# leonsick/s2d

Measured on AMD Instinct MI355X. Metric: clip-frames/sec fwd+loss, R50 M2F-Video T=8 720p Q=100, higher is better.
Workload: dtype f32 (f16x3 MFMA for dense contractions); 1 GPU; KDVideoMaskFormer fwd+loss (student+teacher fwd, GT+KD VideoSetCriterion), c4: 2 clips/GPU x T=8 x 720x1280, Q=100, P=160000, N=10 sparse GT instances/clip, encoder dropout 0.3; clips_per_gpu=2, frames_per_clip=8, parallelism=dp1 (clips sharded, no collective), streams=2

## Files before the change

### s2d_amd/csrc/ffn.hip

```cpp
#include "common.h"
#include "dropout.h"
#include <stdlib.h>
#include <type_traits>

#ifndef S2D_FFN_DBG
#define S2D_FFN_DBG 0
#endif
#if !(S2D_FFN_DBG & 16)
#define FFN_STAMP(slot) do { } while (0)
#endif
#ifndef S2D_FFN_EPI
#define S2D_FFN_EPI 1
#endif
#ifndef S2D_FFN_POSTV
#define S2D_FFN_POSTV 0
#endif

#if S2D_FFN_DBG & 16
__device__ unsigned long long g_ffn_stamps[16 * 4096];
#define FFN_STAMP(slot) do { if (tid == 0 && blockIdx.x < 4096) g_ffn_stamps[16 * blockIdx.x + (slot)] = __builtin_amdgcn_s_memtime(); } while (0)
extern "C" int s2d_ffn_dbg_stamps(unsigned long long *host_out)
{
    return hipMemcpyFromSymbol(host_out, HIP_SYMBOL(g_ffn_stamps), sizeof(g_ffn_stamps)) == hipSuccess ? 0 : -1;
}
#endif

namespace {

typedef _Float16 f16x8 __attribute__((ext_vector_type(8)));
typedef __fp16 h16x2 __attribute__((ext_vector_type(2)));
typedef float f32x2 __attribute__((ext_vector_type(2)));
typedef unsigned int u32x4 __attribute__((ext_vector_type(4)));

constexpr int FC = 256;
constexpr int FRAG = 1024;
constexpr int PART = 32 * FRAG;
constexpr int CHUNKB = 2 * PART;
constexpr int LDS_B1 = 2 * CHUNKB;
constexpr int FMAX = 2048;
constexpr int LDS_PB = LDS_B1 + FMAX * 4;
constexpr int LDS_LN = LDS_PB + FC * 4;

__host__ __device__ __forceinline__ int perm_row(int rho) { return 16 * ((rho >> 2) & 1) + 4 * (rho >> 3) + (rho & 3); }

__device__ __forceinline__ unsigned int pk_hi(float a, float b) { return __builtin_bit_cast(unsigned int, __builtin_amdgcn_cvt_pkrtz(a, b)); }
__device__ __forceinline__ unsigned int pk_lo(float a, float b, unsigned int hi)
{
    const h16x2 h = __builtin_bit_cast(h16x2, hi);
    return __builtin_bit_cast(unsigned int, __builtin_amdgcn_cvt_pkrtz(__builtin_fmaf((float)h[0], -2048.f, a * 2048.f), __builtin_fmaf((float)h[1], -2048.f, b * 2048.f)));
}

__device__ __forceinline__ int lane16_asm()
{
    int v;
    asm volatile("v_mbcnt_lo_u32_b32 %0, -1, 0\n\tv_mbcnt_hi_u32_b32 %0, -1, %0\n\tv_lshlrev_b32 %0, 4, %0" : "=v"(v));
    return v;
}
struct MfmaPrev { f16x8 a, b; };
__device__ __forceinline__ void mfma_a(f32x16 &c, const f16x8 a, const f16x8 b) { c = __builtin_amdgcn_mfma_f32_32x32x16_f16(a, b, c, 0, 0, 0); }
__device__ __forceinline__ void mfma_v(f32x16 &c, const f16x8 a, const f16x8 b, MfmaPrev &pv)
{
    asm("v_mfma_f32_32x32x16_f16 %0, %1, %2, %0" : "+v"(c) : "v"(a), "v"(b), "v"(pv.a), "v"(pv.b));
    pv.a = a; pv.b = b;
}
__device__ __forceinline__ void mfma_v0(f32x16 &c, const f16x8 a, const f16x8 b, MfmaPrev &pv)
{
    asm("v_mfma_f32_32x32x16_f16 %0, %1, %2, 0" : "=&v"(c) : "v"(a), "v"(b), "v"(pv.a), "v"(pv.b));
    pv.a = a; pv.b = b;
}

__host__ __device__ __forceinline__ int kcol(int ks, int h) { return 32 * (ks >> 1) + 16 * h + 8 * (ks & 1); }

__global__ __launch_bounds__(256) void ffn_pack_kernel(const float *__restrict__ W1, const float *__restrict__ W2, int F,
                                                       const float *__restrict__ Wpost, int npost, const float *__restrict__ Wpre, int npre,
                                                       u32x4 *__restrict__ out)
{
    const long gid = (long)blockIdx.x * 256 + threadIdx.x;
    const long nfrag = (long)(F / 32) * 64 + (long)((npost + npre) / 32) * 32;
    if (gid >= nfrag * 64) return;
    const int lane = (int)(gid & 63);
    const long fidx = gid >> 6;
    const int r = lane & 31, h = lane >> 5;
    const float *src;
    int lo;
    if (fidx < (long)(F / 32) * 64) {
        const int frag = (int)(fidx & 63);
        const long c = fidx >> 6;
        lo = frag & 1;
        if (frag < 32) src = W1 + (32 * c + perm_row(r)) * FC + kcol(frag >> 1, h);
        else {
            const int f2 = frag - 32, s = f2 >> 4, t = (f2 >> 1) & 7;
            src = W2 + (long)(32 * t + perm_row(r)) * F + 32 * c + 16 * h + 8 * s;
        }
    } else {
        const long f2 = fidx - (long)(F / 32) * 64;
        const int frag = (int)(f2 & 31);
        lo = frag & 1;
        const long part = f2 >> 5;
        src = (part < npost / 32 ? Wpost + (32 * part + perm_row(r)) * FC : Wpre + (32 * (part - npost / 32) + perm_row(r)) * FC) + kcol(frag >> 1, h);
    }
    u32x4 w;
#pragma unroll
    for (int q = 0; q < 4; ++q) {
        const unsigned int hi = pk_hi(src[2 * q], src[2 * q + 1]);
        w[q] = lo ? pk_lo(src[2 * q], src[2 * q + 1], hi) : hi;
    }
    out[gid] = w;
}

struct FfnParams {
    const float *X;
    float *Y;
    float *Xn;
    int M, nchunks;
    const unsigned int *pack;
    const float *b1, *b2;
    const float *g1, *be1;
    const float *g2, *be2;
    float eps;
    unsigned int thresh;
    float dscale;
    unsigned int k0, k1, site_h, site_o, row0;
    const float *post_bias, *post_pos;
    const float *pre_bias, *pre_res;
    unsigned int site_pre;
    float *post_out;
    int post_parts, post_S, post_npos, post_ld, post_ldpos;
};

template <bool DROP, bool LN1, bool LN2, bool POST, bool PRE>
__global__ __launch_bounds__(256) __attribute__((amdgpu_waves_per_eu(1, 1))) void ffn_f16x3_kernel(FfnParams p)
{
    extern __shared__ __attribute__((aligned(16))) unsigned char lds[];
    const int tid = threadIdx.x, lane = tid & 63, wave = __builtin_amdgcn_readfirstlane(tid >> 6);
#if S2D_FFN_DBG & 16
    const unsigned long long st_te = __builtin_amdgcn_s_memtime();
#endif
    const int tok = lane & 31, h = lane >> 5;
    const long row = (long)blockIdx.x * 128 + wave * 32 + tok;
    const bool rowok = row < p.M;
    const long rowc = rowok ? row : p.M - 1;
    const unsigned int mrow = p.row0 + (unsigned int)rowc;

    const __amdgpu_buffer_rsrc_t rsW = __builtin_amdgcn_make_buffer_rsrc(const_cast<unsigned int *>(p.pack), 0, p.nchunks * CHUNKB + (p.post_parts + (PRE ? 8 : 0)) * PART, 0x00020000);
    auto dma_part = [&](int src_byte, int dst_byte, auto n_) {
        constexpr int n = decltype(n_)::value;
        const int voff = lane16_asm();
#pragma unroll
        for (int i = 0; i < n; ++i) {
            const int piece = wave * n + i;
            __builtin_amdgcn_raw_ptr_buffer_load_lds(rsW, (__attribute__((address_space(3))) void *)(lds + dst_byte + piece * FRAG), 16,
                                                     voff, src_byte + piece * FRAG, 0, 0);
        }
    };
    uint32_t rb[4], rt = 0u;
    f16x8 fr[4][2];
    const unsigned char *lane_lds = lds + lane * 16;
    constexpr int dbg = S2D_FFN_DBG;

    auto philox_half = [&](int idx) {
        const int r = idx >> 1;
        if (!(idx & 1)) {
            const uint64_t pr = (uint64_t)0xCD9E8D57u * rb[2];
            rt = (uint32_t)(pr >> 32) ^ rb[1] ^ (p.k0 + 0x9E3779B9u * (uint32_t)r);
            rb[1] = (uint32_t)pr;
        } else {
            const uint64_t pr = (uint64_t)0xD2511F53u * rb[0];
            rb[2] = (uint32_t)(pr >> 32) ^ rb[3] ^ (p.k1 + 0xBB67AE85u * (uint32_t)r);
            rb[3] = (uint32_t)pr;
            rb[0] = rt;
        }
    };
    auto philox_gap = [&](int g) {
        if (g < 40 && !(g & 1)) philox_half(g >> 1);
    };
    auto dma_piece = [&](int src_byte, int dst_byte) {
        __builtin_amdgcn_raw_ptr_buffer_load_lds(rsW, (__attribute__((address_space(3))) void *)(lds + dst_byte), 16, lane16_asm(), src_byte, 0, 0);
    };
    int voff_loop = 0;
    auto dma_piece4 = [&](int src_byte, int dst_byte, auto sub_, bool in_loop = false) {
        constexpr int SUB = decltype(sub_)::value;
        __builtin_amdgcn_raw_ptr_buffer_load_lds(rsW, (__attribute__((address_space(3))) void *)(lds + dst_byte), 16, in_loop ? voff_loop : lane16_asm(), src_byte, SUB * FRAG, 0);
    };
    auto frag_read = [&](int slot, const unsigned char *at) {
        if (dbg & 8) return;
        fr[slot][0] = *reinterpret_cast<const f16x8 *>(at);
        fr[slot][1] = *reinterpret_cast<const f16x8 *>(at + FRAG);
    };

    const int pre_base = p.nchunks * CHUNKB + p.post_parts * PART;
    auto chunk_loop_prologue = [&](auto w1_) {
        if (decltype(w1_)::value) dma_part(0, 0, std::integral_constant<int, 8>{});
        dma_part(PART, 2 * PART, std::integral_constant<int, 4>{});
        if (decltype(w1_)::value) dma_part((p.nchunks > 1 ? 1 : 0) * CHUNKB, PART, std::integral_constant<int, 8>{});
        for (int i = tid; i < PART / 2 / 16; i += 256)
            reinterpret_cast<u32x4 *>(lds + 3 * PART + PART / 2)[i] = u32x4{0u, 0u, 0u, 0u};
    };
    if (PRE) {
        dma_part(pre_base, 0, std::integral_constant<int, 8>{});
        dma_part(pre_base + PART, PART, std::integral_constant<int, 8>{});
    } else chunk_loop_prologue(std::true_type{});
    {
        auto dma_vec = [&](const float *src, int nbytes, int dst_byte, int first) {
            const __amdgpu_buffer_rsrc_t rs = __builtin_amdgcn_make_buffer_rsrc(const_cast<float *>(src), 0, nbytes, 0x00020000);
            for (int k = 0; k * 1024 < nbytes; ++k)
                if (((first + k) & 3) == wave)
                    __builtin_amdgcn_raw_ptr_buffer_load_lds(rs, (__attribute__((address_space(3))) void *)(lds + dst_byte + k * 1024), 16, lane16_asm(), k * 1024, 0, 0);
        };
        dma_vec(p.b1, p.nchunks * 32 * 4, LDS_B1, 0);
        if (PRE) dma_vec(p.pre_bias, FC * 4, LDS_PB, 1);
        if (LN1) { dma_vec(p.g1, FC * 4, LDS_LN, 2); dma_vec(p.be1, FC * 4, LDS_LN + FC * 4, 3); }
        if (LN2) { dma_vec(p.g2, FC * 4, LDS_LN + 2 * FC * 4, 0); dma_vec(p.be2, FC * 4, LDS_LN + 3 * FC * 4, 1); }
    }

    f32x16 ym[8], yx[8];
    f16x8 xh[16], xl[16];
    float mean1 = 0.f, rstd1 = 1.f;
    auto tile_to_frags = [&](const f32x16 (&src)[8]) {
#pragma unroll
        for (int t = 0; t < 8; ++t)
#pragma unroll
            for (int s2 = 0; s2 < 2; ++s2) {
                u32x4 hi, lo;
#pragma unroll
                for (int q = 0; q < 4; ++q) {
                    const float a = src[t][8 * s2 + 2 * q], b = src[t][8 * s2 + 2 * q + 1];
                    hi[q] = pk_hi(a, b);
                    lo[q] = pk_lo(a, b, hi[q]);
                }
                xh[2 * t + s2] = __builtin_bit_cast(f16x8, hi);
                xl[2 * t + s2] = __builtin_bit_cast(f16x8, lo);
            }
    };
    {
        const float *xr = p.X + rowc * FC + 16 * h;
#pragma unroll
        for (int t = 0; t < 8; ++t)
#pragma unroll
            for (int q = 0; q < 4; ++q) {
                const f32x4 a = (dbg & 512) ? f32x4{(float)lane, 1.f, (float)t, (float)q} : *reinterpret_cast<const f32x4 *>(xr + 32 * t + 4 * q);
                f32x16 &dst = PRE ? yx[t] : ym[t];
                dst[4 * q] = a[0]; dst[4 * q + 1] = a[1]; dst[4 * q + 2] = a[2]; dst[4 * q + 3] = a[3];
            }
        if constexpr (PRE) {
            const float *resr = p.pre_res + rowc * FC + 16 * h;
#pragma unroll
            for (int t = 0; t < 8; ++t)
#pragma unroll
                for (int q = 0; q < 4; ++q) {
                    const f32x4 a = (dbg & 256) ? f32x4{0.f, 0.f, 0.f, 0.f} : *reinterpret_cast<const f32x4 *>(resr + 32 * t + 4 * q);
                    ym[t][4 * q] = a[0]; ym[t][4 * q + 1] = a[1]; ym[t][4 * q + 2] = a[2]; ym[t][4 * q + 3] = a[3];
                }
            __builtin_amdgcn_sched_barrier(0);
            tile_to_frags(yx);
            FFN_STAMP(7);
            const unsigned char *pbo = lds + LDS_PB + 64 * h;
            f32x16 qm[2], qx[2], zero16, binit;
#pragma unroll
            for (int r = 0; r < 16; ++r) zero16[r] = 0.f;
            uint32_t mk[4];
            auto bias_init = [&](int t) {
#pragma unroll
                for (int q = 0; q < 4; ++q) {
                    const f32x4 v = *reinterpret_cast<const f32x4 *>(pbo + 128 * t + 16 * q);
#pragma unroll
                    for (int e = 0; e < 4; ++e) binit[4 * q + e] = v[e];
                }
            };
            auto pre_out = [&](const f32x16 &m, const f32x16 &x, auto t_, int q) {
                constexpr int T = decltype(t_)::value;
#pragma unroll
                for (int e = 0; e < 4; ++e) {
                    float v = __builtin_fmaf(x[4 * q + e], 1.0f / 2048.0f, m[4 * q + e]);
                    if (DROP) v *= ((mk[q] >> (8 * e)) & 0xFFu) >= p.thresh ? p.dscale : 0.f;
                    ym[T][4 * q + e] += v;
                }
            };
            auto pre_part = [&](auto j_) {
                constexpr int J = decltype(j_)::value, CUR = J & 1;
                const unsigned char *w = lane_lds + (J & 3) * PART, *wn = lane_lds + ((J + 1) & 3) * PART;
                const int src2 = J + 2 < 8 ? pre_base + (J + 2) * PART : (J == 6 || p.nchunks < 2 ? 0 : CHUNKB), dst2 = ((J + 2) & 3) * PART;
                if (DROP) { rb[0] = mrow; rb[1] = (uint32_t)(2 * J + h); rb[2] = p.site_pre; rb[3] = 0u; }
#pragma unroll
                for (int ks = 0; ks < 16; ++ks) {
                    const int sl = ks & 3, sn = (ks + 2) & 3;
                    if (ks == 14) {
                        asm volatile("s_waitcnt vmcnt(8) lgkmcnt(0)" ::: "memory");
                        __builtin_amdgcn_s_barrier();
                        __builtin_amdgcn_sched_barrier(0);
                        if (DROP) {
#pragma unroll
                            for (int c = 0; c < 4; ++c) mk[c] = rb[c];
                        }
                        if (J < 7) bias_init(J + 1);
                    }
                    frag_read(sn, ks < 14 ? w + (2 * ks + 4) * FRAG : wn + (2 * (ks - 14)) * FRAG);
                    if (ks == 0) qm[CUR] = __builtin_amdgcn_mfma_f32_32x32x16_f16(fr[sl][0], xh[ks], binit, 0, 0, 0); else mfma_a(qm[CUR], fr[sl][0], xh[ks]);
                    if (DROP) philox_gap(3 * ks);
                    __builtin_amdgcn_sched_barrier(0);
                    if (ks == 0) qx[CUR] = __builtin_amdgcn_mfma_f32_32x32x16_f16(fr[sl][0], xl[ks], zero16, 0, 0, 0); else mfma_a(qx[CUR], fr[sl][0], xl[ks]);
                    if (ks < 8) {
                        const int s4 = src2 + (wave * 8 + (ks & 4)) * FRAG, d4 = dst2 + (wave * 8 + (ks & 4)) * FRAG;
                        switch (ks & 3) {
                        case 0: dma_piece4(s4, d4, std::integral_constant<int, 0>{}); break;
                        case 1: dma_piece4(s4, d4, std::integral_constant<int, 1>{}); break;
                        case 2: dma_piece4(s4, d4, std::integral_constant<int, 2>{}); break;
                        default: dma_piece4(s4, d4, std::integral_constant<int, 3>{}); break;
                        }
                    }
                    if (DROP) philox_gap(3 * ks + 1);
                    __builtin_amdgcn_sched_barrier(0);
                    mfma_a(qx[CUR], fr[sl][1], xh[ks]);
                    if (J > 0 && ks >= 6 && ks < 14 && !(ks & 1)) pre_out(qm[CUR ^ 1], qx[CUR ^ 1], std::integral_constant<int, (J > 0 ? J - 1 : 0)>{}, (ks - 6) >> 1);
                    if (DROP) philox_gap(3 * ks + 2);
                    __builtin_amdgcn_sched_barrier(0);
                }
            };
            asm volatile("s_waitcnt vmcnt(0)" ::: "memory");
            __syncthreads();
            frag_read(0, lane_lds);
            frag_read(1, lane_lds + 2 * FRAG);
            bias_init(0);
            pre_part(std::integral_constant<int, 0>{}); pre_part(std::integral_constant<int, 1>{});
            pre_part(std::integral_constant<int, 2>{}); pre_part(std::integral_constant<int, 3>{});
            pre_part(std::integral_constant<int, 4>{}); pre_part(std::integral_constant<int, 5>{});
            pre_part(std::integral_constant<int, 6>{}); pre_part(std::integral_constant<int, 7>{});
#pragma unroll
            for (int q = 0; q < 4; ++q) pre_out(qm[1], qx[1], std::integral_constant<int, 7>{}, q);
            asm volatile("s_waitcnt lgkmcnt(0)" ::: "memory");
            __syncthreads();
            FFN_STAMP(8);
            chunk_loop_prologue(std::false_type{});
        }
        if (LN1) {
            if (!PRE) { asm volatile("s_waitcnt vmcnt(0)" ::: "memory"); __syncthreads(); }
            float s = 0.f;
#pragma unroll
            for (int t = 0; t < 8; ++t)
#pragma unroll
                for (int r = 0; r < 16; ++r) s += ym[t][r];
            s += __shfl_xor(s, 32, 64);
            mean1 = s / (float)FC;
            float ss = 0.f;
#pragma unroll
            for (int t = 0; t < 8; ++t)
#pragma unroll
                for (int r = 0; r < 16; ++r) { const float d = ym[t][r] - mean1; ss += d * d; }
            ss += __shfl_xor(ss, 32, 64);
            rstd1 = 1.f / sqrtf(ss / (float)FC + p.eps);
#pragma unroll
            for (int t = 0; t < 8; ++t)
#pragma unroll
                for (int q = 0; q < 4; ++q) {
                    const float *lnp = reinterpret_cast<const float *>(lds + LDS_LN) + 32 * t + 16 * h + 4 * q;
                    const f32x4 ga = *reinterpret_cast<const f32x4 *>(lnp), be = *reinterpret_cast<const f32x4 *>(lnp + FC);
                    f32x4 v = {ym[t][4 * q], ym[t][4 * q + 1], ym[t][4 * q + 2], ym[t][4 * q + 3]};
                    v = (v - mean1) * rstd1 * ga + be;
                    ym[t][4 * q] = v[0]; ym[t][4 * q + 1] = v[1]; ym[t][4 * q + 2] = v[2]; ym[t][4 * q + 3] = v[3];
                    if (((PRE && S2D_FFN_EPI != 1) || (p.Xn && rowok)) && !(dbg & 128)) *reinterpret_cast<f32x4 *>(p.Xn + rowc * FC + 32 * t + 16 * h + 4 * q) = v;
                }
        }
        tile_to_frags(ym);
        FFN_STAMP(9);
    }

#pragma unroll
    for (int t = 0; t < 8; ++t) {
#pragma unroll
        for (int q = 0; q < 4; ++q) {
            const f32x4 b = *reinterpret_cast<const f32x4 *>(p.b2 + 32 * t + 16 * h + 4 * q);
            ym[t][4 * q] = b[0]; ym[t][4 * q + 1] = b[1]; ym[t][4 * q + 2] = b[2]; ym[t][4 * q + 3] = b[3];
        }
#pragma unroll
        for (int r = 0; r < 16; ++r) yx[t][r] = 0.f;
    }

    f32x16 am, ax;
    u32x4 hw[2], lw[2];
    float hv0 = 0.f, hv1 = 0.f;
    MfmaPrev pv;
    pv.a = xh[0]; pv.b = xh[0];
    unsigned int hhi = 0u;

    auto hquarter = [&](int s, int idx) {
        const int q = idx >> 2, part = idx & 3, r0 = 8 * s + 2 * q;
        if (part == 0) {
            hv0 = fmaxf(__builtin_fmaf(ax[r0], 1.0f / 2048.0f, am[r0]), 0.f);
            hv1 = fmaxf(__builtin_fmaf(ax[r0 + 1], 1.0f / 2048.0f, am[r0 + 1]), 0.f);
        } else if (part == 1) {
            if (DROP) {
                const uint32_t w = rb[2 * s + (q >> 1)];
                hv0 *= ((w >> (16 * (q & 1))) & 0xFFu) >= p.thresh ? p.dscale : 0.f;
                hv1 *= ((w >> (16 * (q & 1) + 8)) & 0xFFu) >= p.thresh ? p.dscale : 0.f;
            }
        } else if (part == 2) {
            hhi = pk_hi(hv0, hv1);
            hw[s][q] = hhi;
        } else {
            lw[s][q] = pk_lo(hv0, hv1, hhi);
        }
    };
    auto dma_k = [&](int k, int pc) {
        const int cur = pc & 1, last = p.nchunks - 1;
        if (dbg & 1) return;
        auto go = [&](int src, int dst) {
            switch (k & 3) {
            case 0: dma_piece4(src, dst, std::integral_constant<int, 0>{}, true); break;
            case 1: dma_piece4(src, dst, std::integral_constant<int, 1>{}, true); break;
            case 2: dma_piece4(src, dst, std::integral_constant<int, 2>{}, true); break;
            default: dma_piece4(src, dst, std::integral_constant<int, 3>{}, true); break;
            }
        };
        if (k < 8) go(min(pc + 2, last) * CHUNKB + (wave * 8 + (k & 4)) * FRAG, cur * PART + (wave * 8 + (k & 4)) * FRAG);
        else if (k < 12) go(min(pc + 1, last) * CHUNKB + PART + wave * 4 * FRAG, 2 * PART + (cur ^ 1) * (PART / 2) + wave * 4 * FRAG);
        else go(pc * CHUNKB + PART + PART / 2 + wave * 4 * FRAG, 3 * PART + cur * (PART / 2) + wave * 4 * FRAG);
    };
    auto bias_read = [&](int pc) {
        const float *bp = reinterpret_cast<const float *>(lds + LDS_B1) + 32 * pc + 16 * h;
#pragma unroll
        for (int q = 0; q < 4; ++q) {
            const f32x4 b = *reinterpret_cast<const f32x4 *>(bp + 4 * q);
            am[4 * q] = b[0]; am[4 * q + 1] = b[1]; am[4 * q + 2] = b[2]; am[4 * q + 3] = b[3];
        }
    };
    auto post_gap = [&](int j, int pc) {
        if (j % 3 == 1 && j / 3 < 16) dma_k(j / 3, pc);
    };
    auto gemm2_pass = [&](auto s_, const unsigned char *wf, const unsigned char *next, int j0, int pc, int first_q, int bias_pc) {
        constexpr int S = decltype(s_)::value;
        const f16x8 bh = __builtin_bit_cast(f16x8, hw[S]), bl = __builtin_bit_cast(f16x8, lw[S]);
#pragma unroll
        for (int t = 0; t < 8; ++t) {
            const int sl = t & 3, sn = (t + 2) & 3;
            frag_read(sn, t + 2 < 8 ? wf + (2 * t + 4) * FRAG : next + (2 * (t + 2 - 8)) * FRAG);
            mfma_a(ym[t], fr[sl][0], bh);
            post_gap(j0 + 3 * t, pc);
            if (3 * t >= first_q && 3 * t < first_q + 16 && !(dbg & 4)) hquarter(S ^ 1, 3 * t - first_q);
            __builtin_amdgcn_sched_barrier(0);
            mfma_a(yx[t], fr[sl][0], bl);
            post_gap(j0 + 3 * t + 1, pc);
            if (3 * t + 1 >= first_q && 3 * t + 1 < first_q + 16 && !(dbg & 4)) hquarter(S ^ 1, 3 * t + 1 - first_q);
            __builtin_amdgcn_sched_barrier(0);
            mfma_a(yx[t], fr[sl][1], bh);
            post_gap(j0 + 3 * t + 2, pc);
            if (3 * t + 2 >= first_q && 3 * t + 2 < first_q + 16 && !(dbg & 4)) hquarter(S ^ 1, 3 * t + 2 - first_q);
            if (S == 0 && t == 6) bias_read(bias_pc);
            __builtin_amdgcn_sched_barrier(0);
        }
    };

    hw[1] = u32x4{0u, 0u, 0u, 0u}; lw[1] = hw[1];
    asm volatile("s_waitcnt vmcnt(0)" ::: "memory");
    __syncthreads();
    frag_read(0, lane_lds);
    frag_read(1, lane_lds + 2 * FRAG);
    bias_read(0);
    voff_loop = lane16_asm();
#if S2D_FFN_DBG & 16
    const unsigned long long st_t0 = __builtin_amdgcn_s_memtime(), st_r0 = __builtin_amdgcn_s_memrealtime();
#endif
    for (int pc = 0; pc < p.nchunks; ++pc) {
        const int cur = pc & 1;
        const unsigned char *w1 = lane_lds + cur * PART;
        const unsigned char *w2a = lane_lds + 3 * PART + (cur ^ 1) * (PART / 2);
        const unsigned char *w2b = lane_lds + 2 * PART + cur * (PART / 2);
        if (DROP) { rb[0] = mrow; rb[1] = (uint32_t)(2 * pc + h); rb[2] = p.site_h; rb[3] = 0u; }
#pragma unroll
        for (int ks = 0; ks < 16; ++ks) {
            const int sl = ks & 3, sn = (ks + 2) & 3;
            if (ks == 14) {
                asm volatile("s_waitcnt vmcnt(0) lgkmcnt(0)" ::: "memory");
                if (!(dbg & 2)) __builtin_amdgcn_s_barrier();
                __builtin_amdgcn_sched_barrier(0);
            }
            frag_read(sn, ks < 14 ? w1 + (2 * ks + 4) * FRAG : w2a + (2 * (ks - 14)) * FRAG);
            mfma_v(am, fr[sl][0], xh[ks], pv);
            if (ks >= 14) post_gap(3 * (ks - 14), pc);
            if (DROP) philox_gap(3 * ks);
            __builtin_amdgcn_sched_barrier(0);
            if (ks == 0) mfma_v0(ax, fr[sl][0], xl[ks], pv); else mfma_v(ax, fr[sl][0], xl[ks], pv);
            if (ks >= 14) post_gap(3 * (ks - 14) + 1, pc);
            if (DROP) philox_gap(3 * ks + 1);
            __builtin_amdgcn_sched_barrier(0);
            mfma_v(ax, fr[sl][1], xh[ks], pv);
            if (ks >= 14) post_gap(3 * (ks - 14) + 2, pc);
            if (DROP) philox_gap(3 * ks + 2);
            __builtin_amdgcn_sched_barrier(0);
        }
        gemm2_pass(std::integral_constant<int, 1>{}, w2a, w2b, 6, pc, 6, -1);
        gemm2_pass(std::integral_constant<int, 0>{}, w2b, lane_lds + (cur ^ 1) * PART, 30, pc, 2, pc + 1 < p.nchunks ? pc + 1 : pc);
    }
#if S2D_FFN_DBG & 16
    {
        const unsigned long long st_t1 = __builtin_amdgcn_s_memtime(), st_r1 = __builtin_amdgcn_s_memrealtime();
        if (tid == 0 && blockIdx.x < 4096) {
            g_ffn_stamps[16 * blockIdx.x] = st_te;
            g_ffn_stamps[16 * blockIdx.x + 1] = st_t0; g_ffn_stamps[16 * blockIdx.x + 2] = st_r0;
            g_ffn_stamps[16 * blockIdx.x + 3] = st_t1; g_ffn_stamps[16 * blockIdx.x + 4] = st_r1;
        }
    }
#endif
    asm volatile("s_waitcnt vmcnt(0) lgkmcnt(0)" ::: "memory");
    __syncthreads();
    const int post_base = p.nchunks * CHUNKB;
    if (POST) {
#pragma unroll
        for (int k = 0; k < 8; ++k) dma_piece(post_base + (wave * 8 + k) * FRAG, (wave * 8 + k) * FRAG);
#pragma unroll
        for (int k = 0; k < 8; ++k) dma_piece(post_base + (p.post_parts > 1 ? PART : 0) + (wave * 8 + k) * FRAG, PART + (wave * 8 + k) * FRAG);
    }
    f32x4 resv[8][4];
    const float *rsrc = (PRE ? p.Xn : p.X) + rowc * FC + 16 * h;
    if (S2D_FFN_EPI == 2) {
#pragma unroll
        for (int t = 0; t < 8; ++t)
#pragma unroll
            for (int q = 0; q < 4; ++q) resv[t][q] = (dbg & 64) ? f32x4{0.f, 0.f, 0.f, 0.f} : *reinterpret_cast<const f32x4 *>(rsrc + 32 * t + 4 * q);
        __builtin_amdgcn_sched_barrier(0);
    }
    frag_read(0, lane_lds + 3 * PART + ((p.nchunks - 1) & 1) * (PART / 2));
    frag_read(1, lane_lds + 3 * PART + ((p.nchunks - 1) & 1) * (PART / 2) + 2 * FRAG);
    gemm2_pass(std::integral_constant<int, 1>{}, lane_lds + 3 * PART + ((p.nchunks - 1) & 1) * (PART / 2), lane_lds, 1000, 0, 1000, -1);

    FFN_STAMP(10);
    asm volatile("s_nop 15\n\ts_nop 15\n\ts_nop 15\n\ts_nop 15" ::: "memory");
    float s = 0.f;
#pragma unroll
    for (int t = 0; t < 8; ++t) {
        uint32_t m0[4];
        if (DROP) s2d_philox4x32_10(mrow, (uint32_t)(2 * t + h), p.site_o, 0u, p.k0, p.k1, m0);
#pragma unroll
        for (int q = 0; q < 4; ++q) {
            f32x4 x;
            if (S2D_FFN_EPI == 2) x = resv[t][q];
            else if (S2D_FFN_EPI == 0) x = (dbg & 64) ? f32x4{0.f, 0.f, 0.f, 0.f} : *reinterpret_cast<const f32x4 *>(rsrc + 32 * t + 4 * q);
            else {
#pragma unroll
                for (int e = 0; e < 4; ++e) {
                    const int r = 4 * q + e;
                    x[e] = (dbg & 64) ? 0.f : __builtin_fmaf((float)xl[2 * t + (r >> 3)][r & 7], 1.0f / 2048.0f, (float)xh[2 * t + (r >> 3)][r & 7]);
                }
            }
            if (LN1 && !PRE && S2D_FFN_EPI != 1) {
                const float *lnp = reinterpret_cast<const float *>(lds + LDS_LN) + 32 * t + 16 * h + 4 * q;
                const f32x4 ga = *reinterpret_cast<const f32x4 *>(lnp), be = *reinterpret_cast<const f32x4 *>(lnp + FC);
                x = (x - mean1) * rstd1 * ga + be;
            }
#pragma unroll
            for (int e = 0; e < 4; ++e) {
                const int r = 4 * q + e;
                float v = ym[t][r] + yx[t][r] * (1.0f / 2048.0f);
                if (DROP) v = ((m0[q] >> (8 * e)) & 0xFFu) >= p.thresh ? v * p.dscale : 0.f;
                v += x[e];
                ym[t][r] = v;
                s += v;
            }
        }
        __builtin_amdgcn_sched_barrier(0);
    }
    FFN_STAMP(11);
    float mean = 0.f, rstd = 1.f;
    if (LN2) {
        s += __shfl_xor(s, 32, 64);
        mean = s / (float)FC;
        float ss = 0.f;
#pragma unroll
        for (int t = 0; t < 8; ++t)
#pragma unroll
            for (int r = 0; r < 16; ++r) { const float d = ym[t][r] - mean; ss += d * d; }
        ss += __shfl_xor(ss, 32, 64);
        rstd = 1.f / sqrtf(ss / (float)FC + p.eps);
    }
    float *yr = p.Y + rowc * FC + 16 * h;
#pragma unroll
    for (int t = 0; t < 8; ++t) {
#pragma unroll
        for (int q = 0; q < 4; ++q) {
            f32x4 v = {ym[t][4 * q], ym[t][4 * q + 1], ym[t][4 * q + 2], ym[t][4 * q + 3]};
            if (LN2) {
                const float *lnp = reinterpret_cast<const float *>(lds + LDS_LN) + 2 * FC + 32 * t + 16 * h + 4 * q;
                const f32x4 ga = *reinterpret_cast<const f32x4 *>(lnp), be = *reinterpret_cast<const f32x4 *>(lnp + FC);
                v = (v - mean) * rstd * ga + be;
            }
            if (rowok && !(dbg & 128)) *reinterpret_cast<f32x4 *>(yr + 32 * t + 4 * q) = v;
            if (POST) { ym[t][4 * q] = v[0]; ym[t][4 * q + 1] = v[1]; ym[t][4 * q + 2] = v[2]; ym[t][4 * q + 3] = v[3]; }
        }
        __builtin_amdgcn_sched_barrier(0);
    }
#if S2D_FFN_DBG & 16
    if (tid == 0 && blockIdx.x < 4096) g_ffn_stamps[16 * blockIdx.x + 5] = __builtin_amdgcn_s_memtime();
#endif
    if constexpr (POST) {
        tile_to_frags(ym);
        const long prow = rowc % p.post_S;
        const float *posr = p.post_pos + prow * p.post_ldpos + 16 * h;
        float *outr = p.post_out + rowc * p.post_ld + 16 * h;
        const float *pbr = p.post_bias + 16 * h;
        f32x16 pm[2], px[2], zero16;
#pragma unroll
        for (int r = 0; r < 16; ++r) zero16[r] = 0.f;
        f32x4 pos4[4];
        auto add_load = [&](int j, bool haspos) {
#pragma unroll
            for (int q = 0; q < 4; ++q) pos4[q] = *reinterpret_cast<const f32x4 *>((haspos ? posr : pbr) + 32 * j + 4 * q);
        };
        auto tile_out = [&](const f32x16 &m, const f32x16 &x, int j, int q) {
            f32x4 v = {m[4 * q] + x[4 * q] * (1.0f / 2048.0f), m[4 * q + 1] + x[4 * q + 1] * (1.0f / 2048.0f),
                       m[4 * q + 2] + x[4 * q + 2] * (1.0f / 2048.0f), m[4 * q + 3] + x[4 * q + 3] * (1.0f / 2048.0f)};
            v += pos4[q];
            if (!(dbg & 32)) *reinterpret_cast<f32x4 *>(outr + 32 * j + 4 * q) = v;
        };
        auto post_part = [&](auto cur_, auto prev_, int j) {
            constexpr int CUR = decltype(cur_)::value, PREV = decltype(prev_)::value;
            const unsigned char *w = lane_lds + (j & 3) * PART, *wn = lane_lds + ((j + 1) & 3) * PART;
            const int last = p.post_parts - 1;
            const int src2 = post_base + min(j + 2, last) * PART, dst2 = ((j + 2) & 3) * PART;
#pragma unroll
            for (int ks = 0; ks < 16; ++ks) {
                const int sl = ks & 3, sn = (ks + 2) & 3;
                if (ks == 14) {
                    if (PREV) { if (S2D_FFN_POSTV) asm volatile("s_waitcnt vmcnt(20) lgkmcnt(0)" ::: "memory"); else asm volatile("s_waitcnt vmcnt(16) lgkmcnt(0)" ::: "memory"); }
                    else asm volatile("s_waitcnt vmcnt(8) lgkmcnt(0)" ::: "memory");
                    __builtin_amdgcn_s_barrier();
                    __builtin_amdgcn_sched_barrier(0);
                }
                frag_read(sn, ks < 14 ? w + (2 * ks + 4) * FRAG : wn + (2 * (ks - 14)) * FRAG);
                if (ks == 0) pm[CUR] = __builtin_amdgcn_mfma_f32_32x32x16_f16(fr[sl][0], xh[ks], zero16, 0, 0, 0); else mfma_a(pm[CUR], fr[sl][0], xh[ks]);
                if (ks == 0 && PREV) add_load(j - 1, PREV == 1);
                __builtin_amdgcn_sched_barrier(0);
                if (ks == 0) px[CUR] = __builtin_amdgcn_mfma_f32_32x32x16_f16(fr[sl][0], xl[ks], zero16, 0, 0, 0); else mfma_a(px[CUR], fr[sl][0], xl[ks]);
                auto piece = [&](int k) {
                    const int s4 = src2 + (wave * 8 + (k & 4)) * FRAG, d4 = dst2 + (wave * 8 + (k & 4)) * FRAG;
                    switch (k & 3) {
                    case 0: dma_piece4(s4, d4, std::integral_constant<int, 0>{}); break;
                    case 1: dma_piece4(s4, d4, std::integral_constant<int, 1>{}); break;
                    case 2: dma_piece4(s4, d4, std::integral_constant<int, 2>{}); break;
                    default: dma_piece4(s4, d4, std::integral_constant<int, 3>{}); break;
                    }
                };
                if (S2D_FFN_POSTV) { if (ks < 4) piece(2 * ks); }
                else if (ks < 8) piece(ks);
                __builtin_amdgcn_sched_barrier(0);
                mfma_a(px[CUR], fr[sl][1], xh[ks]);
                if (S2D_FFN_POSTV && ks < 4) piece(2 * ks + 1);
                if (PREV && ks >= 6 && ks < 14 && !(ks & 1)) tile_out(pm[CUR ^ 1], px[CUR ^ 1], j - 1, (ks - 6) >> 1);
                __builtin_amdgcn_sched_barrier(0);
            }
        };
        typedef std::integral_constant<int, 0> I0;
        typedef std::integral_constant<int, 1> I1;
        typedef std::integral_constant<int, 2> I2;
        asm volatile("s_waitcnt vmcnt(0)" ::: "memory");
        __syncthreads();
        frag_read(0, lane_lds);
        frag_read(1, lane_lds + 2 * FRAG);
        const int npt = p.post_npos >> 5;
        post_part(I0{}, I0{}, 0);
        for (int j = 1; j < p.post_parts; ++j) {
            if (j == 4) FFN_STAMP(13);
            if (j == 8) FFN_STAMP(14);
            if (j == 12) FFN_STAMP(15);
            const bool hp = j - 1 < npt;
            if (j & 1) { if (hp) post_part(I1{}, I1{}, j); else post_part(I1{}, I2{}, j); }
            else { if (hp) post_part(I0{}, I1{}, j); else post_part(I0{}, I2{}, j); }
        }
        {
            const int j = p.post_parts - 1;
            add_load(j, j < npt);
#pragma unroll
            for (int q = 0; q < 4; ++q) { if (j & 1) tile_out(pm[1], px[1], j, q); else tile_out(pm[0], px[0], j, q); }
        }
    }
#if S2D_FFN_DBG & 16
    asm volatile("s_waitcnt vmcnt(0)" ::: "memory");
    if (tid == 0 && blockIdx.x < 4096) g_ffn_stamps[16 * blockIdx.x + 6] = __builtin_amdgcn_s_memtime();
#endif
}

}

extern "C" {

long s2d_ffn_pack_words(int C, int F, int Npost, int pre)
{
    if (C != FC || F <= 0 || F % 32 || F > FMAX || Npost < 0 || Npost % 32 || Npost > 4096 || (pre != 0 && pre != 1)) return -1;
    return (long)(F / 32) * (CHUNKB / 4) + (long)(Npost / 32 + (pre ? FC / 32 : 0)) * (PART / 4);
}

int s2d_ffn_pack_f16(const float *W1, const float *W2, int C, int F, const float *Wpost, int Npost, const float *Wpre, void *out,
                     hipStream_t stream)
{
    if (s2d_ffn_pack_words(C, F, Npost, Wpre != nullptr) < 0 || !W1 || !W2 || !out || (Npost > 0 && !Wpost)) return S2D_ERR_ARG;
    const int npre = Wpre ? FC : 0;
    const long n = ((long)(F / 32) * 64 + (long)((Npost + npre) / 32) * 32) * 64;
    hipLaunchKernelGGL(ffn_pack_kernel, dim3(cdiv(n, 256)), dim3(256), 0, stream, W1, W2, F, Wpost, Npost, Wpre, npre,
                       reinterpret_cast<u32x4 *>(out));
    S2D_CHECK_LAUNCH();
    return S2D_OK;
}

int s2d_ffn_fused_f32(const float *x, long M, int C, int F, const void *pack, const float *b1, const float *b2, const float *ln1_gamma,
                      const float *ln1_beta, const float *ln2_gamma, const float *ln2_beta, float eps, float p, uint64_t seed,
                      unsigned site_hidden, unsigned site_out, unsigned row0, float *xn, float *y, int Npost, const float *post_bias,
                      const float *post_pos, int post_S, int post_npos, long post_ldpos, float *post_out, long post_ld,
                      const float *pre_bias, const float *pre_res, unsigned site_pre, hipStream_t stream)
{
    if (s2d_ffn_pack_words(C, F, Npost, pre_bias != nullptr) < 0 || !x || !pack || !b1 || !b2 || !y || M <= 0 || M > 0x7FFFFF00L) return S2D_ERR_ARG;
    if ((ln1_gamma == nullptr) != (ln1_beta == nullptr) || (ln2_gamma == nullptr) != (ln2_beta == nullptr)) return S2D_ERR_ARG;
    for (const void *q16 : {(const void *)b1, (const void *)ln1_gamma, (const void *)ln1_beta, (const void *)ln2_gamma, (const void *)ln2_beta, (const void *)pre_bias})
        if (reinterpret_cast<uintptr_t>(q16) & 15) return S2D_ERR_ARG;
    if (xn && !ln1_gamma) return S2D_ERR_ARG;
    if (!(p >= 0.f && p < 1.f)) return S2D_ERR_ARG;
    if (pre_bias && (!pre_res || (!xn && S2D_FFN_EPI != 1) || !ln1_gamma || !ln2_gamma)) return S2D_ERR_ARG;
    if (Npost > 0 && (!post_bias || !post_out || post_ld < Npost || (post_ld & 3) || post_npos < 0 || post_npos > Npost || (post_npos & 31) ||
                      (post_npos > 0 && (!post_pos || post_S <= 0 || post_ldpos < post_npos || (post_ldpos & 3))) || M * post_ld > 0x7FFFFFFFL * 4))
        return S2D_ERR_ARG;
    FfnParams q;
    q.X = x; q.Y = y; q.Xn = xn; q.M = (int)M; q.nchunks = F / 32;
    q.pack = reinterpret_cast<const unsigned int *>(pack);
    q.b1 = b1; q.b2 = b2; q.g1 = ln1_gamma; q.be1 = ln1_beta; q.g2 = ln2_gamma; q.be2 = ln2_beta; q.eps = eps;
    q.thresh = s2d_dropout_thresh(p);
    q.dscale = q.thresh ? s2d_dropout_scale(q.thresh) : 1.f;
    q.k0 = (unsigned int)seed; q.k1 = (unsigned int)(seed >> 32); q.site_h = site_hidden; q.site_o = site_out; q.row0 = row0;
    q.post_bias = post_bias; q.post_pos = post_npos > 0 ? post_pos : post_bias; q.post_out = post_out; q.post_parts = Npost / 32;
    q.pre_bias = pre_bias; q.pre_res = pre_res; q.site_pre = site_pre;
    q.post_S = post_npos > 0 ? post_S : 1; q.post_npos = post_npos; q.post_ld = (int)post_ld; q.post_ldpos = (int)post_ldpos;
    const int smem = LDS_LN + 4 * FC * 4;
    const dim3 grid(cdiv(M, 128)), block(256);
    static S2dDevOnce attr[32];
    const bool drop = q.thresh != 0, ln1 = ln1_gamma != nullptr, ln2 = ln2_gamma != nullptr, post = Npost > 0, pre = pre_bias != nullptr;
    const void *fn = nullptr;
#define S2D_FFN_CASE(D, A, B, P, R) if (drop == D && ln1 == A && ln2 == B && post == P && pre == R) fn = (const void *)ffn_f16x3_kernel<D, A, B, P, R>;
    S2D_FFN_CASE(false, false, false, false, false) S2D_FFN_CASE(false, false, true, false, false) S2D_FFN_CASE(false, true, true, false, false)
    S2D_FFN_CASE(true, false, false, false, false) S2D_FFN_CASE(true, false, true, false, false) S2D_FFN_CASE(true, true, true, false, false)
    S2D_FFN_CASE(false, true, true, true, false) S2D_FFN_CASE(true, true, true, true, false)
    S2D_FFN_CASE(false, true, true, false, true) S2D_FFN_CASE(true, true, true, false, true)
    S2D_FFN_CASE(false, true, true, true, true) S2D_FFN_CASE(true, true, true, true, true)
#undef S2D_FFN_CASE
    if (!fn) return S2D_ERR_ARG;
    const int slot = (pre ? 16 : 0) + (post ? 8 : 0) + (drop ? 4 : 0) + (ln1 ? 2 : 0) + (ln2 ? 1 : 0);
    if (!attr[slot].done()) {
        if (hipFuncSetAttribute(fn, hipFuncAttributeMaxDynamicSharedMemorySize, smem) != hipSuccess) return S2D_ERR_LAUNCH;
        attr[slot].mark();
    }
    void *args[] = {&q};
    if (hipLaunchKernel(fn, grid, block, args, smem, stream) != hipSuccess) return S2D_ERR_LAUNCH;
    S2D_CHECK_LAUNCH();
    return S2D_OK;
}

}
```

Before: 176.0 clip-frames/s.

## Restructure FFN kernel to 16x16 MFMA tiles with two workgroups per CU

Rewrites the fused FFN f16x3 kernel from 32x32x16 MFMA tiles at 128 rows per workgroup and one wave per EU to 16x16x32 MFMA tiles at 64 rows per workgroup. The weight staging buffer shrinks from four parts to a simple double buffer so two workgroups fit per CU. The hand-scheduled asm MFMA pipeline with inline Philox and interleaved DMA is replaced by a plain per-part loop that waits, syncs and prefetches the next part, with Philox masks computed per 8 columns. The weight pack layout changes to match. This trades the careful software pipelining and larger tiles for more occupancy and simpler code, so it risks more barriers, more weight reloads per row and exposed DMA latency.

```diff
diff --git a/s2d_amd/csrc/ffn.hip b/s2d_amd/csrc/ffn.hip
--- a/s2d_amd/csrc/ffn.hip
+++ b/s2d_amd/csrc/ffn.hip
@@ -9,12 +9,7 @@
 #if !(S2D_FFN_DBG & 16)
 #define FFN_STAMP(slot) do { } while (0)
 #endif
-#ifndef S2D_FFN_EPI
 #define S2D_FFN_EPI 1
-#endif
-#ifndef S2D_FFN_POSTV
-#define S2D_FFN_POSTV 0
-#endif
 
 #if S2D_FFN_DBG & 16
 __device__ unsigned long long g_ffn_stamps[16 * 4096];
@@ -29,19 +24,21 @@
 
 typedef _Float16 f16x8 __attribute__((ext_vector_type(8)));
 typedef __fp16 h16x2 __attribute__((ext_vector_type(2)));
-typedef float f32x2 __attribute__((ext_vector_type(2)));
 typedef unsigned int u32x4 __attribute__((ext_vector_type(4)));
 
 constexpr int FC = 256;
 constexpr int FRAG = 1024;
 constexpr int PART = 32 * FRAG;
 constexpr int CHUNKB = 2 * PART;
-constexpr int LDS_B1 = 2 * CHUNKB;
+constexpr int LDS_B1 = 2 * PART;
 constexpr int FMAX = 2048;
 constexpr int LDS_PB = LDS_B1 + FMAX * 4;
 constexpr int LDS_LN = LDS_PB + FC * 4;
-
-__host__ __device__ __forceinline__ int perm_row(int rho) { return 16 * ((rho >> 2) & 1) + 4 * (rho >> 3) + (rho & 3); }
+constexpr int LDS_ALL = LDS_LN + 4 * FC * 4;
+static_assert(2 * LDS_ALL <= 160 * 1024, "two workgroups per CU");
+constexpr int ROWS_WG = 64;
+
+__host__ __device__ __forceinline__ int perm_row(int tau, int rho) { return 8 * (rho >> 2) + 4 * tau + (rho & 3); }
 
 __device__ __forceinline__ unsigned int pk_hi(float a, float b) { return __builtin_bit_cast(unsigned int, __builtin_amdgcn_cvt_pkrtz(a, b)); }
 __device__ __forceinline__ unsigned int pk_lo(float a, float b, unsigned int hi)
@@ -49,27 +46,18 @@
     const h16x2 h = __builtin_bit_cast(h16x2, hi);
     return __builtin_bit_cast(unsigned int, __builtin_amdgcn_cvt_pkrtz(__builtin_fmaf((float)h[0], -2048.f, a * 2048.f), __builtin_fmaf((float)h[1], -2048.f, b * 2048.f)));
 }
-
-__device__ __forceinline__ int lane16_asm()
-{
-    int v;
-    asm volatile("v_mbcnt_lo_u32_b32 %0, -1, 0\n\tv_mbcnt_hi_u32_b32 %0, -1, %0\n\tv_lshlrev_b32 %0, 4, %0" : "=v"(v));
-    return v;
-}
-struct MfmaPrev { f16x8 a, b; };
-__device__ __forceinline__ void mfma_a(f32x16 &c, const f16x8 a, const f16x8 b) { c = __builtin_amdgcn_mfma_f32_32x32x16_f16(a, b, c, 0, 0, 0); }
-__device__ __forceinline__ void mfma_v(f32x16 &c, const f16x8 a, const f16x8 b, MfmaPrev &pv)
-{
-    asm("v_mfma_f32_32x32x16_f16 %0, %1, %2, %0" : "+v"(c) : "v"(a), "v"(b), "v"(pv.a), "v"(pv.b));
-    pv.a = a; pv.b = b;
-}
-__device__ __forceinline__ void mfma_v0(f32x16 &c, const f16x8 a, const f16x8 b, MfmaPrev &pv)
-{
-    asm("v_mfma_f32_32x32x16_f16 %0, %1, %2, 0" : "=&v"(c) : "v"(a), "v"(b), "v"(pv.a), "v"(pv.b));
-    pv.a = a; pv.b = b;
-}
-
-__host__ __device__ __forceinline__ int kcol(int ks, int h) { return 32 * (ks >> 1) + 16 * h + 8 * (ks & 1); }
+__device__ __forceinline__ void mask8(uint32_t row, uint32_t col8, uint32_t site, uint32_t k0, uint32_t k1, uint32_t &w0, uint32_t &w1)
+{
+    uint32_t r[4];
+    s2d_philox4x32_10(row, col8 >> 1, site, 0u, k0, k1, r);
+    w0 = (col8 & 1u) ? r[2] : r[0];
+    w1 = (col8 & 1u) ? r[3] : r[1];
+}
+__device__ __forceinline__ float mask_mul(uint32_t w0, uint32_t w1, int e, uint32_t thresh, float scale)
+{
+    return (((e < 4 ? w0 : w1) >> (8 * (e & 3))) & 0xFFu) >= thresh ? scale : 0.f;
+}
+__device__ __forceinline__ void mfma(f32x4 &c, const f16x8 a, const f16x8 b) { c = __builtin_amdgcn_mfma_f32_16x16x32_f16(a, b, c, 0, 0, 0); }
 
 __global__ __launch_bounds__(256) void ffn_pack_kernel(const float *__restrict__ W1, const float *__restrict__ W2, int F,
                                                        const float *__restrict__ Wpost, int npost, const float *__restrict__ Wpre, int npre,
@@ -80,30 +68,28 @@
     if (gid >= nfrag * 64) return;
     const int lane = (int)(gid & 63);
     const long fidx = gid >> 6;
-    const int r = lane & 31, h = lane >> 5;
+    const int rho = lane & 15, g = lane >> 4;
     const float *src;
-    int lo;
+    int f;
     if (fidx < (long)(F / 32) * 64) {
         const int frag = (int)(fidx & 63);
         const long c = fidx >> 6;
-        lo = frag & 1;
-        if (frag < 32) src = W1 + (32 * c + perm_row(r)) * FC + kcol(frag >> 1, h);
-        else {
-            const int f2 = frag - 32, s = f2 >> 4, t = (f2 >> 1) & 7;
-            src = W2 + (long)(32 * t + perm_row(r)) * F + 32 * c + 16 * h + 8 * s;
-        }
+        f = frag & 31;
+        const int tau = (f >> 1) & 1, idx = f >> 2;
+        if (frag < 32) src = W1 + (32 * c + perm_row(tau, rho)) * FC + 32 * idx + 8 * g;
+        else src = W2 + (long)(32 * idx + perm_row(tau, rho)) * F + 32 * c + 8 * g;
     } else {
         const long f2 = fidx - (long)(F / 32) * 64;
-        const int frag = (int)(f2 & 31);
-        lo = frag & 1;
+        f = (int)(f2 & 31);
+        const int tau = (f >> 1) & 1, idx = f >> 2;
         const long part = f2 >> 5;
-        src = (part < npost / 32 ? Wpost + (32 * part + perm_row(r)) * FC : Wpre + (32 * (part - npost / 32) + perm_row(r)) * FC) + kcol(frag >> 1, h);
+        src = (part < npost / 32 ? Wpost + (32 * part + perm_row(tau, rho)) * FC : Wpre + (32 * (part - npost / 32) + perm_row(tau, rho)) * FC) + 32 * idx + 8 * g;
     }
     u32x4 w;
 #pragma unroll
     for (int q = 0; q < 4; ++q) {
         const unsigned int hi = pk_hi(src[2 * q], src[2 * q + 1]);
-        w[q] = lo ? pk_lo(src[2 * q], src[2 * q + 1], hi) : hi;
+        w[q] = (f & 1) ? pk_lo(src[2 * q], src[2 * q + 1], hi) : hi;
     }
     out[gid] = w;
 }
@@ -129,83 +115,44 @@
 };
 
 template <bool DROP, bool LN1, bool LN2, bool POST, bool PRE>
-__global__ __launch_bounds__(256) __attribute__((amdgpu_waves_per_eu(1, 1))) void ffn_f16x3_kernel(FfnParams p)
+__global__ __launch_bounds__(256, 2) void ffn_f16x3_kernel(FfnParams p)
 {
     extern __shared__ __attribute__((aligned(16))) unsigned char lds[];
     const int tid = threadIdx.x, lane = tid & 63, wave = __builtin_amdgcn_readfirstlane(tid >> 6);
 #if S2D_FFN_DBG & 16
     const unsigned long long st_te = __builtin_amdgcn_s_memtime();
 #endif
-    const int tok = lane & 31, h = lane >> 5;
-    const long row = (long)blockIdx.x * 128 + wave * 32 + tok;
+    const int tok = lane & 15, g = lane >> 4;
+    const long row = (long)blockIdx.x * ROWS_WG + wave * 16 + tok;
     const bool rowok = row < p.M;
     const long rowc = rowok ? row : p.M - 1;
     const unsigned int mrow = p.row0 + (unsigned int)rowc;
-
-    const __amdgpu_buffer_rsrc_t rsW = __builtin_amdgcn_make_buffer_rsrc(const_cast<unsigned int *>(p.pack), 0, p.nchunks * CHUNKB + (p.post_parts + (PRE ? 8 : 0)) * PART, 0x00020000);
-    auto dma_part = [&](int src_byte, int dst_byte, auto n_) {
-        constexpr int n = decltype(n_)::value;
-        const int voff = lane16_asm();
-#pragma unroll
-        for (int i = 0; i < n; ++i) {
-            const int piece = wave * n + i;
-            __builtin_amdgcn_raw_ptr_buffer_load_lds(rsW, (__attribute__((address_space(3))) void *)(lds + dst_byte + piece * FRAG), 16,
-                                                     voff, src_byte + piece * FRAG, 0, 0);
-        }
+    const int cb = 8 * g;
+
+    const int nparts = (PRE ? 8 : 0) + 2 * p.nchunks + p.post_parts;
+    const int pre_base = (2 * p.nchunks + p.post_parts) * PART;
+    const __amdgpu_buffer_rsrc_t rsW = __builtin_amdgcn_make_buffer_rsrc(const_cast<unsigned int *>(p.pack), 0, nparts * PART, 0x00020000);
+    const int voff = lane * 16;
+    auto part_src = [&](int n) { return PRE ? (n < 8 ? pre_base + n * PART : (n - 8) * PART) : n * PART; };
+    auto dma_part = [&](int n) {
+        const int src = part_src(n) + wave * 8 * FRAG, dst = (n & 1) * PART + wave * 8 * FRAG;
+#pragma unroll
+        for (int i = 0; i < 8; ++i)
+            __builtin_amdgcn_raw_ptr_buffer_load_lds(rsW, (__attribute__((address_space(3))) void *)(lds + dst + i * FRAG), 16, voff, src + i * FRAG, 0, 0);
     };
-    uint32_t rb[4], rt = 0u;
-    f16x8 fr[4][2];
-    const unsigned char *lane_lds = lds + lane * 16;
-    constexpr int dbg = S2D_FFN_DBG;
-
-    auto philox_half = [&](int idx) {
-        const int r = idx >> 1;
-        if (!(idx & 1)) {
-            const uint64_t pr = (uint64_t)0xCD9E8D57u * rb[2];
-            rt = (uint32_t)(pr >> 32) ^ rb[1] ^ (p.k0 + 0x9E3779B9u * (uint32_t)r);
-            rb[1] = (uint32_t)pr;
-        } else {
-            const uint64_t pr = (uint64_t)0xD2511F53u * rb[0];
-            rb[2] = (uint32_t)(pr >> 32) ^ rb[3] ^ (p.k1 + 0xBB67AE85u * (uint32_t)r);
-            rb[3] = (uint32_t)pr;
-            rb[0] = rt;
-        }
+    auto step_begin = [&](int n) -> const unsigned char * {
+        asm volatile("s_waitcnt vmcnt(0)" ::: "memory");
+        __syncthreads();
+        if (n + 1 < nparts) dma_part(n + 1);
+        return lds + (n & 1) * PART + lane * 16;
     };
-    auto philox_gap = [&](int g) {
-        if (g < 40 && !(g & 1)) philox_half(g >> 1);
-    };
-    auto dma_piece = [&](int src_byte, int dst_byte) {
-        __builtin_amdgcn_raw_ptr_buffer_load_lds(rsW, (__attribute__((address_space(3))) void *)(lds + dst_byte), 16, lane16_asm(), src_byte, 0, 0);
-    };
-    int voff_loop = 0;
-    auto dma_piece4 = [&](int src_byte, int dst_byte, auto sub_, bool in_loop = false) {
-        constexpr int SUB = decltype(sub_)::value;
-        __builtin_amdgcn_raw_ptr_buffer_load_lds(rsW, (__attribute__((address_space(3))) void *)(lds + dst_byte), 16, in_loop ? voff_loop : lane16_asm(), src_byte, SUB * FRAG, 0);
-    };
-    auto frag_read = [&](int slot, const unsigned char *at) {
-        if (dbg & 8) return;
-        fr[slot][0] = *reinterpret_cast<const f16x8 *>(at);
-        fr[slot][1] = *reinterpret_cast<const f16x8 *>(at + FRAG);
-    };
-
-    const int pre_base = p.nchunks * CHUNKB + p.post_parts * PART;
-    auto chunk_loop_prologue = [&](auto w1_) {
-        if (decltype(w1_)::value) dma_part(0, 0, std::integral_constant<int, 8>{});
-        dma_part(PART, 2 * PART, std::integral_constant<int, 4>{});
-        if (decltype(w1_)::value) dma_part((p.nchunks > 1 ? 1 : 0) * CHUNKB, PART, std::integral_constant<int, 8>{});
-        for (int i = tid; i < PART / 2 / 16; i += 256)
-            reinterpret_cast<u32x4 *>(lds + 3 * PART + PART / 2)[i] = u32x4{0u, 0u, 0u, 0u};
-    };
-    if (PRE) {
-        dma_part(pre_base, 0, std::integral_constant<int, 8>{});
-        dma_part(pre_base + PART, PART, std::integral_constant<int, 8>{});
-    } else chunk_loop_prologue(std::true_type{});
+    dma_part(0);
     {
         auto dma_vec = [&](const float *src, int nbytes, int dst_byte, int first) {
             const __amdgpu_buffer_rsrc_t rs = __builtin_amdgcn_make_buffer_rsrc(const_cast<float *>(src), 0, nbytes, 0x00020000);
             for (int k = 0; k * 1024 < nbytes; ++k)
                 if (((first + k) & 3) == wave)
-                    __builtin_amdgcn_raw_ptr_buffer_load_lds(rs, (__attribute__((address_space(3))) void *)(lds + dst_byte + k * 1024), 16, lane16_asm(), k * 1024, 0, 0);
+                    __builtin_amdgcn_raw_ptr_buffer_load_lds(rs, (__attribute__((address_space(3))) void *)(lds + dst_byte + k * 1024), 16, voff, k * 1024, 0, 0);
         };
         dma_vec(p.b1, p.nchunks * 32 * 4, LDS_B1, 0);
         if (PRE) dma_vec(p.pre_bias, FC * 4, LDS_PB, 1);
@@ -213,282 +160,139 @@
         if (LN2) { dma_vec(p.g2, FC * 4, LDS_LN + 2 * FC * 4, 0); dma_vec(p.be2, FC * 4, LDS_LN + 3 * FC * 4, 1); }
     }
 
-    f32x16 ym[8], yx[8];
-    f16x8 xh[16], xl[16];
-    float mean1 = 0.f, rstd1 = 1.f;
-    auto tile_to_frags = [&](const f32x16 (&src)[8]) {
-#pragma unroll
-        for (int t = 0; t < 8; ++t)
-#pragma unroll
-            for (int s2 = 0; s2 < 2; ++s2) {
-                u32x4 hi, lo;
-#pragma unroll
-                for (int q = 0; q < 4; ++q) {
-                    const float a = src[t][8 * s2 + 2 * q], b = src[t][8 * s2 + 2 * q + 1];
-                    hi[q] = pk_hi(a, b);
-                    lo[q] = pk_lo(a, b, hi[q]);
+    f32x4 ym[16], yx[16];
+    f16x8 xh[8], xl[8];
+    auto tile_to_frags = [&](const f32x4 (&src)[16]) {
+#pragma unroll
+        for (int t = 0; t < 8; ++t) {
+            u32x4 hi, lo;
+#pragma unroll
+            for (int q = 0; q < 4; ++q) {
+                const float a = src[2 * t + (q >> 1)][2 * (q & 1)], b = src[2 * t + (q >> 1)][2 * (q & 1) + 1];
+                hi[q] = pk_hi(a, b);
+                lo[q] = pk_lo(a, b, hi[q]);
+            }
+            xh[t] = __builtin_bit_cast(f16x8, hi);
+            xl[t] = __builtin_bit_cast(f16x8, lo);
+        }
+    };
+    auto load_tile = [&](const float *base, f32x4 (&dst)[16]) {
+        const float *xr = base + rowc * FC + cb;
+#pragma unroll
+        for (int u = 0; u < 16; ++u) dst[u] = *reinterpret_cast<const f32x4 *>(xr + 32 * (u >> 1) + 4 * (u & 1));
+    };
+    auto xpart = [&](const unsigned char *w, f32x4 (&m)[2], f32x4 (&x)[2]) {
+#pragma unroll
+        for (int ks = 0; ks < 8; ++ks) {
+            const f16x8 h0 = *reinterpret_cast<const f16x8 *>(w + (4 * ks) * FRAG), l0 = *reinterpret_cast<const f16x8 *>(w + (4 * ks + 1) * FRAG);
+            const f16x8 h1 = *reinterpret_cast<const f16x8 *>(w + (4 * ks + 2) * FRAG), l1 = *reinterpret_cast<const f16x8 *>(w + (4 * ks + 3) * FRAG);
+            mfma(m[0], h0, xh[ks]); mfma(x[0], h0, xl[ks]);
+            mfma(m[1], h1, xh[ks]); mfma(x[1], h1, xl[ks]);
+            mfma(x[0], l0, xh[ks]); mfma(x[1], l1, xh[ks]);
+        }
+    };
+    const f32x4 zero4 = {0.f, 0.f, 0.f, 0.f};
+    int n = 0;
+
+    if constexpr (PRE) {
+        load_tile(p.X, yx);
+        load_tile(p.pre_res, ym);
+        tile_to_frags(yx);
+        FFN_STAMP(7);
+#pragma unroll
+        for (int J = 0; J < 8; ++J) {
+            const unsigned char *w = step_begin(n++);
+            f32x4 qm[2], qx[2];
+#pragma unroll
+            for (int tau = 0; tau < 2; ++tau) {
+                qm[tau] = *reinterpret_cast<const f32x4 *>(lds + LDS_PB + (32 * J + cb + 4 * tau) * 4);
+                qx[tau] = zero4;
+            }
+            uint32_t mk0 = 0u, mk1 = 0u;
+            if (DROP) mask8(mrow, (uint32_t)(4 * J + g), p.site_pre, p.k0, p.k1, mk0, mk1);
+            xpart(w, qm, qx);
+#pragma unroll
+            for (int tau = 0; tau < 2; ++tau)
+#pragma unroll
+                for (int i = 0; i < 4; ++i) {
+                    float v = __builtin_fmaf(qx[tau][i], 1.0f / 2048.0f, qm[tau][i]);
+                    if (DROP) v *= mask_mul(mk0, mk1, 4 * tau + i, p.thresh, p.dscale);
+                    ym[2 * J + tau][i] += v;
                 }
-                xh[2 * t + s2] = __builtin_bit_cast(f16x8, hi);
-                xl[2 * t + s2] = __builtin_bit_cast(f16x8, lo);
-            }
-    };
-    {
-        const float *xr = p.X + rowc * FC + 16 * h;
-#pragma unroll
-        for (int t = 0; t < 8; ++t)
-#pragma unroll
-            for (int q = 0; q < 4; ++q) {
-                const f32x4 a = (dbg & 512) ? f32x4{(float)lane, 1.f, (float)t, (float)q} : *reinterpret_cast<const f32x4 *>(xr + 32 * t + 4 * q);
-                f32x16 &dst = PRE ? yx[t] : ym[t];
-                dst[4 * q] = a[0]; dst[4 * q + 1] = a[1]; dst[4 * q + 2] = a[2]; dst[4 * q + 3] = a[3];
-            }
-        if constexpr (PRE) {
-            const float *resr = p.pre_res + rowc * FC + 16 * h;
-#pragma unroll
-            for (int t = 0; t < 8; ++t)
-#pragma unroll
-                for (int q = 0; q < 4; ++q) {
-                    const f32x4 a = (dbg & 256) ? f32x4{0.f, 0.f, 0.f, 0.f} : *reinterpret_cast<const f32x4 *>(resr + 32 * t + 4 * q);
-                    ym[t][4 * q] = a[0]; ym[t][4 * q + 1] = a[1]; ym[t][4 * q + 2] = a[2]; ym[t][4 * q + 3] = a[3];
-                }
-            __builtin_amdgcn_sched_barrier(0);
-            tile_to_frags(yx);
-            FFN_STAMP(7);
-            const unsigned char *pbo = lds + LDS_PB + 64 * h;
-            f32x16 qm[2], qx[2], zero16, binit;
-#pragma unroll
-            for (int r = 0; r < 16; ++r) zero16[r] = 0.f;
-            uint32_t mk[4];
-            auto bias_init = [&](int t) {
-#pragma unroll
-                for (int q = 0; q < 4; ++q) {
-                    const f32x4 v = *reinterpret_cast<const f32x4 *>(pbo + 128 * t + 16 * q);
-#pragma unroll
-                    for (int e = 0; e < 4; ++e) binit[4 * q + e] = v[e];
-                }
-            };
-            auto pre_out = [&](const f32x16 &m, const f32x16 &x, auto t_, int q) {
-                constexpr int T = decltype(t_)::value;
-#pragma unroll
-                for (int e = 0; e < 4; ++e) {
-                    float v = __builtin_fmaf(x[4 * q + e], 1.0f / 2048.0f, m[4 * q + e]);
-                    if (DROP) v *= ((mk[q] >> (8 * e)) & 0xFFu) >= p.thresh ? p.dscale : 0.f;
-                    ym[T][4 * q + e] += v;
-                }
-            };
-            auto pre_part = [&](auto j_) {
-                constexpr int J = decltype(j_)::value, CUR = J & 1;
-                const unsigned char *w = lane_lds + (J & 3) * PART, *wn = lane_lds + ((J + 1) & 3) * PART;
-                const int src2 = J + 2 < 8 ? pre_base + (J + 2) * PART : (J == 6 || p.nchunks < 2 ? 0 : CHUNKB), dst2 = ((J + 2) & 3) * PART;
-                if (DROP) { rb[0] = mrow; rb[1] = (uint32_t)(2 * J + h); rb[2] = p.site_pre; rb[3] = 0u; }
-#pragma unroll
-                for (int ks = 0; ks < 16; ++ks) {
-                    const int sl = ks & 3, sn = (ks + 2) & 3;
-                    if (ks == 14) {
-                        asm volatile("s_waitcnt vmcnt(8) lgkmcnt(0)" ::: "memory");
-                        __builtin_amdgcn_s_barrier();
-                        __builtin_amdgcn_sched_barrier(0);
-                        if (DROP) {
-#pragma unroll
-                            for (int c = 0; c < 4; ++c) mk[c] = rb[c];
-                        }
-                        if (J < 7) bias_init(J + 1);
-                    }
-                    frag_read(sn, ks < 14 ? w + (2 * ks + 4) * FRAG : wn + (2 * (ks - 14)) * FRAG);
-                    if (ks == 0) qm[CUR] = __builtin_amdgcn_mfma_f32_32x32x16_f16(fr[sl][0], xh[ks], binit, 0, 0, 0); else mfma_a(qm[CUR], fr[sl][0], xh[ks]);
-                    if (DROP) philox_gap(3 * ks);
-                    __builtin_amdgcn_sched_barrier(0);
-                    if (ks == 0) qx[CUR] = __builtin_amdgcn_mfma_f32_32x32x16_f16(fr[sl][0], xl[ks], zero16, 0, 0, 0); else mfma_a(qx[CUR], fr[sl][0], xl[ks]);
-                    if (ks < 8) {
-                        const int s4 = src2 + (wave * 8 + (ks & 4)) * FRAG, d4 = dst2 + (wave * 8 + (ks & 4)) * FRAG;
-                        switch (ks & 3) {
-                        case 0: dma_piece4(s4, d4, std::integral_constant<int, 0>{}); break;
-                        case 1: dma_piece4(s4, d4, std::integral_constant<int, 1>{}); break;
-                        case 2: dma_piece4(s4, d4, std::integral_constant<int, 2>{}); break;
-                        default: dma_piece4(s4, d4, std::integral_constant<int, 3>{}); break;
-                        }
-                    }
-                    if (DROP) philox_gap(3 * ks + 1);
-                    __builtin_amdgcn_sched_barrier(0);
-                    mfma_a(qx[CUR], fr[sl][1], xh[ks]);
-                    if (J > 0 && ks >= 6 && ks < 14 && !(ks & 1)) pre_out(qm[CUR ^ 1], qx[CUR ^ 1], std::integral_constant<int, (J > 0 ? J - 1 : 0)>{}, (ks - 6) >> 1);
-                    if (DROP) philox_gap(3 * ks + 2);
-                    __builtin_amdgcn_sched_barrier(0);
-                }
-            };
-            asm volatile("s_waitcnt vmcnt(0)" ::: "memory");
-            __syncthreads();
-            frag_read(0, lane_lds);
-            frag_read(1, lane_lds + 2 * FRAG);
-            bias_init(0);
-            pre_part(std::integral_constant<int, 0>{}); pre_part(std::integral_constant<int, 1>{});
-            pre_part(std::integral_constant<int, 2>{}); pre_part(std::integral_constant<int, 3>{});
-            pre_part(std::integral_constant<int, 4>{}); pre_part(std::integral_constant<int, 5>{});
-            pre_part(std::integral_constant<int, 6>{}); pre_part(std::integral_constant<int, 7>{});
-#pragma unroll
-            for (int q = 0; q < 4; ++q) pre_out(qm[1], qx[1], std::integral_constant<int, 7>{}, q);
-            asm volatile("s_waitcnt lgkmcnt(0)" ::: "memory");
-            __syncthreads();
-            FFN_STAMP(8);
-            chunk_loop_prologue(std::false_type{});
-        }
-        if (LN1) {
-            if (!PRE) { asm volatile("s_waitcnt vmcnt(0)" ::: "memory"); __syncthreads(); }
-            float s = 0.f;
-#pragma unroll
-            for (int t = 0; t < 8; ++t)
-#pragma unroll
-                for (int r = 0; r < 16; ++r) s += ym[t][r];
-            s += __shfl_xor(s, 32, 64);
-            mean1 = s / (float)FC;
-            float ss = 0.f;
-#pragma unroll
-            for (int t = 0; t < 8; ++t)
-#pragma unroll
-                for (int r = 0; r < 16; ++r) { const float d = ym[t][r] - mean1; ss += d * d; }
-            ss += __shfl_xor(ss, 32, 64);
-            rstd1 = 1.f / sqrtf(ss / (float)FC + p.eps);
-#pragma unroll
-            for (int t = 0; t < 8; ++t)
-#pragma unroll
-                for (int q = 0; q < 4; ++q) {
-                    const float *lnp = reinterpret_cast<const float *>(lds + LDS_LN) + 32 * t + 16 * h + 4 * q;
-                    const f32x4 ga = *reinterpret_cast<const f32x4 *>(lnp), be = *reinterpret_cast<const f32x4 *>(lnp + FC);
-                    f32x4 v = {ym[t][4 * q], ym[t][4 * q + 1], ym[t][4 * q + 2], ym[t][4 * q + 3]};
-                    v = (v - mean1) * rstd1 * ga + be;
-                    ym[t][4 * q] = v[0]; ym[t][4 * q + 1] = v[1]; ym[t][4 * q + 2] = v[2]; ym[t][4 * q + 3] = v[3];
-                    if (((PRE && S2D_FFN_EPI != 1) || (p.Xn && rowok)) && !(dbg & 128)) *reinterpret_cast<f32x4 *>(p.Xn + rowc * FC + 32 * t + 16 * h + 4 * q) = v;
-                }
-        }
-        tile_to_frags(ym);
-        FFN_STAMP(9);
-    }
-
-#pragma unroll
-    for (int t = 0; t < 8; ++t) {
+        }
+        FFN_STAMP(8);
+    } else {
+        load_tile(p.X, ym);
+    }
+    if (LN1) {
+        if (!PRE) { asm volatile("s_waitcnt vmcnt(0)" ::: "memory"); __syncthreads(); }
+        float s = 0.f;
+#pragma unroll
+        for (int u = 0; u < 16; ++u)
+#pragma unroll
+            for (int i = 0; i < 4; ++i) s += ym[u][i];
+        s += __shfl_xor(s, 16, 64);
+        s += __shfl_xor(s, 32, 64);
+        const float mean1 = s / (float)FC;
+        float ss = 0.f;
+#pragma unroll
+        for (int u = 0; u < 16; ++u)
+#pragma unroll
+            for (int i = 0; i < 4; ++i) { const float d = ym[u][i] - mean1; ss += d * d; }
+        ss += __shfl_xor(ss, 16, 64);
+        ss += __shfl_xor(ss, 32, 64);
+        const float rstd1 = 1.f / sqrtf(ss / (float)FC + p.eps);
+#pragma unroll
+        for (int u = 0; u < 16; ++u) {
+            const int col = 32 * (u >> 1) + cb + 4 * (u & 1);
+            const float *lnp = reinterpret_cast<const float *>(lds + LDS_LN) + col;
+            const f32x4 ga = *reinterpret_cast<const f32x4 *>(lnp), be = *reinterpret_cast<const f32x4 *>(lnp + FC);
+            ym[u] = (ym[u] - mean1) * rstd1 * ga + be;
+            if (p.Xn && rowok) *reinterpret_cast<f32x4 *>(p.Xn + rowc * FC + col) = ym[u];
+        }
+    }
+    tile_to_frags(ym);
+    FFN_STAMP(9);
+
+#pragma unroll
+    for (int u = 0; u < 16; ++u) {
+        ym[u] = *reinterpret_cast<const f32x4 *>(p.b2 + 32 * (u >> 1) + cb + 4 * (u & 1));
+        yx[u] = zero4;
+    }
+
+#if S2D_FFN_DBG & 16
+    const unsigned long long st_t0 = __builtin_amdgcn_s_memtime(), st_r0 = __builtin_amdgcn_s_memrealtime();
+#endif
+    for (int pc = 0; pc < p.nchunks; ++pc) {
+        const unsigned char *w1 = step_begin(n++);
+        f32x4 am[2], ax[2];
+#pragma unroll
+        for (int tau = 0; tau < 2; ++tau) {
+            am[tau] = *reinterpret_cast<const f32x4 *>(lds + LDS_B1 + (32 * pc + cb + 4 * tau) * 4);
+            ax[tau] = zero4;
+        }
+        uint32_t mk0 = 0u, mk1 = 0u;
+        if (DROP) mask8(mrow, (uint32_t)(4 * pc + g), p.site_h, p.k0, p.k1, mk0, mk1);
+        xpart(w1, am, ax);
+        u32x4 hw, lw;
 #pragma unroll
         for (int q = 0; q < 4; ++q) {
-            const f32x4 b = *reinterpret_cast<const f32x4 *>(p.b2 + 32 * t + 16 * h + 4 * q);
-            ym[t][4 * q] = b[0]; ym[t][4 * q + 1] = b[1]; ym[t][4 * q + 2] = b[2]; ym[t][4 * q + 3] = b[3];
-        }
-#pragma unroll
-        for (int r = 0; r < 16; ++r) yx[t][r] = 0.f;
-    }
-
-    f32x16 am, ax;
-    u32x4 hw[2], lw[2];
-    float hv0 = 0.f, hv1 = 0.f;
-    MfmaPrev pv;
-    pv.a = xh[0]; pv.b = xh[0];
-    unsigned int hhi = 0u;
-
-    auto hquarter = [&](int s, int idx) {
-        const int q = idx >> 2, part = idx & 3, r0 = 8 * s + 2 * q;
-        if (part == 0) {
-            hv0 = fmaxf(__builtin_fmaf(ax[r0], 1.0f / 2048.0f, am[r0]), 0.f);
-            hv1 = fmaxf(__builtin_fmaf(ax[r0 + 1], 1.0f / 2048.0f, am[r0 + 1]), 0.f);
-        } else if (part == 1) {
-            if (DROP) {
-                const uint32_t w = rb[2 * s + (q >> 1)];
-                hv0 *= ((w >> (16 * (q & 1))) & 0xFFu) >= p.thresh ? p.dscale : 0.f;
-                hv1 *= ((w >> (16 * (q & 1) + 8)) & 0xFFu) >= p.thresh ? p.dscale : 0.f;
-            }
-        } else if (part == 2) {
-            hhi = pk_hi(hv0, hv1);
-            hw[s][q] = hhi;
-        } else {
-            lw[s][q] = pk_lo(hv0, hv1, hhi);
-        }
-    };
-    auto dma_k = [&](int k, int pc) {
-        const int cur = pc & 1, last = p.nchunks - 1;
-        if (dbg & 1) return;
-        auto go = [&](int src, int dst) {
-            switch (k & 3) {
-            case 0: dma_piece4(src, dst, std::integral_constant<int, 0>{}, true); break;
-            case 1: dma_piece4(src, dst, std::integral_constant<int, 1>{}, true); break;
-            case 2: dma_piece4(src, dst, std::integral_constant<int, 2>{}, true); break;
-            default: dma_piece4(src, dst, std::integral_constant<int, 3>{}, true); break;
-            }
-        };
-        if (k < 8) go(min(pc + 2, last) * CHUNKB + (wave * 8 + (k & 4)) * FRAG, cur * PART + (wave * 8 + (k & 4)) * FRAG);
-        else if (k < 12) go(min(pc + 1, last) * CHUNKB + PART + wave * 4 * FRAG, 2 * PART + (cur ^ 1) * (PART / 2) + wave * 4 * FRAG);
-        else go(pc * CHUNKB + PART + PART / 2 + wave * 4 * FRAG, 3 * PART + cur * (PART / 2) + wave * 4 * FRAG);
-    };
-    auto bias_read = [&](int pc) {
-        const float *bp = reinterpret_cast<const float *>(lds + LDS_B1) + 32 * pc + 16 * h;
-#pragma unroll
-        for (int q = 0; q < 4; ++q) {
-            const f32x4 b = *reinterpret_cast<const f32x4 *>(bp + 4 * q);
-            am[4 * q] = b[0]; am[4 * q + 1] = b[1]; am[4 * q + 2] = b[2]; am[4 * q + 3] = b[3];
-        }
-    };
-    auto post_gap = [&](int j, int pc) {
-        if (j % 3 == 1 && j / 3 < 16) dma_k(j / 3, pc);
-    };
-    auto gemm2_pass = [&](auto s_, const unsigned char *wf, const unsigned char *next, int j0, int pc, int first_q, int bias_pc) {
-        constexpr int S = decltype(s_)::value;
-        const f16x8 bh = __builtin_bit_cast(f16x8, hw[S]), bl = __builtin_bit_cast(f16x8, lw[S]);
-#pragma unroll
-        for (int t = 0; t < 8; ++t) {
-            const int sl = t & 3, sn = (t + 2) & 3;
-            frag_read(sn, t + 2 < 8 ? wf + (2 * t + 4) * FRAG : next + (2 * (t + 2 - 8)) * FRAG);
-            mfma_a(ym[t], fr[sl][0], bh);
-            post_gap(j0 + 3 * t, pc);
-            if (3 * t >= first_q && 3 * t < first_q + 16 && !(dbg & 4)) hquarter(S ^ 1, 3 * t - first_q);
-            __builtin_amdgcn_sched_barrier(0);
-            mfma_a(yx[t], fr[sl][0], bl);
-            post_gap(j0 + 3 * t + 1, pc);
-            if (3 * t + 1 >= first_q && 3 * t + 1 < first_q + 16 && !(dbg & 4)) hquarter(S ^ 1, 3 * t + 1 - first_q);
-            __builtin_amdgcn_sched_barrier(0);
-            mfma_a(yx[t], fr[sl][1], bh);
-            post_gap(j0 + 3 * t + 2, pc);
-            if (3 * t + 2 >= first_q && 3 * t + 2 < first_q + 16 && !(dbg & 4)) hquarter(S ^ 1, 3 * t + 2 - first_q);
-            if (S == 0 && t == 6) bias_read(bias_pc);
-            __builtin_amdgcn_sched_barrier(0);
-        }
-    };
-
-    hw[1] = u32x4{0u, 0u, 0u, 0u}; lw[1] = hw[1];
-    asm volatile("s_waitcnt vmcnt(0)" ::: "memory");
-    __syncthreads();
-    frag_read(0, lane_lds);
-    frag_read(1, lane_lds + 2 * FRAG);
-    bias_read(0);
-    voff_loop = lane16_asm();
-#if S2D_FFN_DBG & 16
-    const unsigned long long st_t0 = __builtin_amdgcn_s_memtime(), st_r0 = __builtin_amdgcn_s_memrealtime();
-#endif
-    for (int pc = 0; pc < p.nchunks; ++pc) {
-        const int cur = pc & 1;
-        const unsigned char *w1 = lane_lds + cur * PART;
-        const unsigned char *w2a = lane_lds + 3 * PART + (cur ^ 1) * (PART / 2);
-        const unsigned char *w2b = lane_lds + 2 * PART + cur * (PART / 2);
-        if (DROP) { rb[0] = mrow; rb[1] = (uint32_t)(2 * pc + h); rb[2] = p.site_h; rb[3] = 0u; }
-#pragma unroll
-        for (int ks = 0; ks < 16; ++ks) {
-            const int sl = ks & 3, sn = (ks + 2) & 3;
-            if (ks == 14) {
-                asm volatile("s_waitcnt vmcnt(0) lgkmcnt(0)" ::: "memory");
-                if (!(dbg & 2)) __builtin_amdgcn_s_barrier();
-                __builtin_amdgcn_sched_barrier(0);
-            }
-            frag_read(sn, ks < 14 ? w1 + (2 * ks + 4) * FRAG : w2a + (2 * (ks - 14)) * FRAG);
-            mfma_v(am, fr[sl][0], xh[ks], pv);
-            if (ks >= 14) post_gap(3 * (ks - 14), pc);
-            if (DROP) philox_gap(3 * ks);
-            __builtin_amdgcn_sched_barrier(0);
-            if (ks == 0) mfma_v0(ax, fr[sl][0], xl[ks], pv); else mfma_v(ax, fr[sl][0], xl[ks], pv);
-            if (ks >= 14) post_gap(3 * (ks - 14) + 1, pc);
-            if (DROP) philox_gap(3 * ks + 1);
-            __builtin_amdgcn_sched_barrier(0);
-            mfma_v(ax, fr[sl][1], xh[ks], pv);
-            if (ks >= 14) post_gap(3 * (ks - 14) + 2, pc);
-            if (DROP) philox_gap(3 * ks + 2);
-            __builtin_amdgcn_sched_barrier(0);
-        }
-        gemm2_pass(std::integral_constant<int, 1>{}, w2a, w2b, 6, pc, 6, -1);
-        gemm2_pass(std::integral_constant<int, 0>{}, w2b, lane_lds + (cur ^ 1) * PART, 30, pc, 2, pc + 1 < p.nchunks ? pc + 1 : pc);
+            float hv0 = fmaxf(__builtin_fmaf(ax[q >> 1][2 * (q & 1)], 1.0f / 2048.0f, am[q >> 1][2 * (q & 1)]), 0.f);
+            float hv1 = fmaxf(__builtin_fmaf(ax[q >> 1][2 * (q & 1) + 1], 1.0f / 2048.0f, am[q >> 1][2 * (q & 1) + 1]), 0.f);
+            if (DROP) { hv0 *= mask_mul(mk0, mk1, 2 * q, p.thresh, p.dscale); hv1 *= mask_mul(mk0, mk1, 2 * q + 1, p.thresh, p.dscale); }
+            hw[q] = pk_hi(hv0, hv1);
+            lw[q] = pk_lo(hv0, hv1, hw[q]);
+        }
+        const f16x8 bh = __builtin_bit_cast(f16x8, hw), bl = __builtin_bit_cast(f16x8, lw);
+        const unsigned char *w2 = step_begin(n++);
+#pragma unroll
+        for (int u = 0; u < 16; u += 2) {
+            const f16x8 h0 = *reinterpret_cast<const f16x8 *>(w2 + (2 * u) * FRAG), l0 = *reinterpret_cast<const f16x8 *>(w2 + (2 * u + 1) * FRAG);
+            const f16x8 h1 = *reinterpret_cast<const f16x8 *>(w2 + (2 * u + 2) * FRAG), l1 = *reinterpret_cast<const f16x8 *>(w2 + (2 * u + 3) * FRAG);
+            mfma(ym[u], h0, bh); mfma(yx[u], h0, bl);
+            mfma(ym[u + 1], h1, bh); mfma(yx[u + 1], h1, bl);
+            mfma(yx[u], l0, bh); mfma(yx[u + 1], l1, bh);
+        }
     }
 #if S2D_FFN_DBG & 16
     {
@@ -500,92 +304,46 @@
         }
     }
 #endif
-    asm volatile("s_waitcnt vmcnt(0) lgkmcnt(0)" ::: "memory");
-    __syncthreads();
-    const int post_base = p.nchunks * CHUNKB;
-    if (POST) {
-#pragma unroll
-        for (int k = 0; k < 8; ++k) dma_piece(post_base + (wave * 8 + k) * FRAG, (wave * 8 + k) * FRAG);
-#pragma unroll
-        for (int k = 0; k < 8; ++k) dma_piece(post_base + (p.post_parts > 1 ? PART : 0) + (wave * 8 + k) * FRAG, PART + (wave * 8 + k) * FRAG);
-    }
-    f32x4 resv[8][4];
-    const float *rsrc = (PRE ? p.Xn : p.X) + rowc * FC + 16 * h;
-    if (S2D_FFN_EPI == 2) {
-#pragma unroll
-        for (int t = 0; t < 8; ++t)
-#pragma unroll
-            for (int q = 0; q < 4; ++q) resv[t][q] = (dbg & 64) ? f32x4{0.f, 0.f, 0.f, 0.f} : *reinterpret_cast<const f32x4 *>(rsrc + 32 * t + 4 * q);
-        __builtin_amdgcn_sched_barrier(0);
-    }
-    frag_read(0, lane_lds + 3 * PART + ((p.nchunks - 1) & 1) * (PART / 2));
-    frag_read(1, lane_lds + 3 * PART + ((p.nchunks - 1) & 1) * (PART / 2) + 2 * FRAG);
-    gemm2_pass(std::integral_constant<int, 1>{}, lane_lds + 3 * PART + ((p.nchunks - 1) & 1) * (PART / 2), lane_lds, 1000, 0, 1000, -1);
-
-    FFN_STAMP(10);
-    asm volatile("s_nop 15\n\ts_nop 15\n\ts_nop 15\n\ts_nop 15" ::: "memory");
+
     float s = 0.f;
 #pragma unroll
     for (int t = 0; t < 8; ++t) {
-        uint32_t m0[4];
-        if (DROP) s2d_philox4x32_10(mrow, (uint32_t)(2 * t + h), p.site_o, 0u, p.k0, p.k1, m0);
-#pragma unroll
-        for (int q = 0; q < 4; ++q) {
-            f32x4 x;
-            if (S2D_FFN_EPI == 2) x = resv[t][q];
-            else if (S2D_FFN_EPI == 0) x = (dbg & 64) ? f32x4{0.f, 0.f, 0.f, 0.f} : *reinterpret_cast<const f32x4 *>(rsrc + 32 * t + 4 * q);
-            else {
-#pragma unroll
-                for (int e = 0; e < 4; ++e) {
-                    const int r = 4 * q + e;
-                    x[e] = (dbg & 64) ? 0.f : __builtin_fmaf((float)xl[2 * t + (r >> 3)][r & 7], 1.0f / 2048.0f, (float)xh[2 * t + (r >> 3)][r & 7]);
-                }
-            }
-            if (LN1 && !PRE && S2D_FFN_EPI != 1) {
-                const float *lnp = reinterpret_cast<const float *>(lds + LDS_LN) + 32 * t + 16 * h + 4 * q;
-                const f32x4 ga = *reinterpret_cast<const f32x4 *>(lnp), be = *reinterpret_cast<const f32x4 *>(lnp + FC);
-                x = (x - mean1) * rstd1 * ga + be;
-            }
-#pragma unroll
-            for (int e = 0; e < 4; ++e) {
-                const int r = 4 * q + e;
-                float v = ym[t][r] + yx[t][r] * (1.0f / 2048.0f);
-                if (DROP) v = ((m0[q] >> (8 * e)) & 0xFFu) >= p.thresh ? v * p.dscale : 0.f;
-                v += x[e];
-                ym[t][r] = v;
-                s += v;
-            }
-        }
-        __builtin_amdgcn_sched_barrier(0);
+        uint32_t mk0 = 0u, mk1 = 0u;
+        if (DROP) mask8(mrow, (uint32_t)(4 * t + g), p.site_o, p.k0, p.k1, mk0, mk1);
+#pragma unroll
+        for (int e = 0; e < 8; ++e) {
+            const float x = __builtin_fmaf((float)xl[t][e], 1.0f / 2048.0f, (float)xh[t][e]);
+            float v = ym[2 * t + (e >> 2)][e & 3] + yx[2 * t + (e >> 2)][e & 3] * (1.0f / 2048.0f);
+            if (DROP) v *= mask_mul(mk0, mk1, e, p.thresh, p.dscale);
+            v += x;
+            ym[2 * t + (e >> 2)][e & 3] = v;
+            s += v;
+        }
     }
     FFN_STAMP(11);
     float mean = 0.f, rstd = 1.f;
     if (LN2) {
+        s += __shfl_xor(s, 16, 64);
         s += __shfl_xor(s, 32, 64);
         mean = s / (float)FC;
         float ss = 0.f;
 #pragma unroll
-        for (int t = 0; t < 8; ++t)
-#pragma unroll
-            for (int r = 0; r < 16; ++r) { const float d = ym[t][r] - mean; ss += d * d; }
+        for (int u = 0; u < 16; ++u)
+#pragma unroll
+            for (int i = 0; i < 4; ++i) { const float d = ym[u][i] - mean; ss += d * d; }
+        ss += __shfl_xor(ss, 16, 64);
         ss += __shfl_xor(ss, 32, 64);
         rstd = 1.f / sqrtf(ss / (float)FC + p.eps);
     }
-    float *yr = p.Y + rowc * FC + 16 * h;
-#pragma unroll
-    for (int t = 0; t < 8; ++t) {
-#pragma unroll
-        for (int q = 0; q < 4; ++q) {
-            f32x4 v = {ym[t][4 * q], ym[t][4 * q + 1], ym[t][4 * q + 2], ym[t][4 * q + 3]};
-            if (LN2) {
-                const float *lnp = reinterpret_cast<const float *>(lds + LDS_LN) + 2 * FC + 32 * t + 16 * h + 4 * q;
-                const f32x4 ga = *reinterpret_cast<const f32x4 *>(lnp), be = *reinterpret_cast<const f32x4 *>(lnp + FC);
-                v = (v - mean) * rstd * ga + be;
-            }
-            if (rowok && !(dbg & 128)) *reinterpret_cast<f32x4 *>(yr + 32 * t + 4 * q) = v;
-            if (POST) { ym[t][4 * q] = v[0]; ym[t][4 * q + 1] = v[1]; ym[t][4 * q + 2] = v[2]; ym[t][4 * q + 3] = v[3]; }
-        }
-        __builtin_amdgcn_sched_barrier(0);
+#pragma unroll
+    for (int u = 0; u < 16; ++u) {
+        const int col = 32 * (u >> 1) + cb + 4 * (u & 1);
+        if (LN2) {
+            const float *lnp = reinterpret_cast<const float *>(lds + LDS_LN) + 2 * FC + col;
+            const f32x4 ga = *reinterpret_cast<const f32x4 *>(lnp), be = *reinterpret_cast<const f32x4 *>(lnp + FC);
+            ym[u] = (ym[u] - mean) * rstd * ga + be;
+        }
+        if (rowok) *reinterpret_cast<f32x4 *>(p.Y + rowc * FC + col) = ym[u];
     }
 #if S2D_FFN_DBG & 16
     if (tid == 0 && blockIdx.x < 4096) g_ffn_stamps[16 * blockIdx.x + 5] = __builtin_amdgcn_s_memtime();
@@ -593,82 +351,27 @@
     if constexpr (POST) {
         tile_to_frags(ym);
         const long prow = rowc % p.post_S;
-        const float *posr = p.post_pos + prow * p.post_ldpos + 16 * h;
-        float *outr = p.post_out + rowc * p.post_ld + 16 * h;
-        const float *pbr = p.post_bias + 16 * h;
-        f32x16 pm[2], px[2], zero16;
-#pragma unroll
-        for (int r = 0; r < 16; ++r) zero16[r] = 0.f;
-        f32x4 pos4[4];
-        auto add_load = [&](int j, bool haspos) {
-#pragma unroll
-            for (int q = 0; q < 4; ++q) pos4[q] = *reinterpret_cast<const f32x4 *>((haspos ? posr : pbr) + 32 * j + 4 * q);
-        };
-        auto tile_out = [&](const f32x16 &m, const f32x16 &x, int j, int q) {
-            f32x4 v = {m[4 * q] + x[4 * q] * (1.0f / 2048.0f), m[4 * q + 1] + x[4 * q + 1] * (1.0f / 2048.0f),
-                       m[4 * q + 2] + x[4 * q + 2] * (1.0f / 2048.0f), m[4 * q + 3] + x[4 * q + 3] * (1.0f / 2048.0f)};
-            v += pos4[q];
-            if (!(dbg & 32)) *reinterpret_cast<f32x4 *>(outr + 32 * j + 4 * q) = v;
-        };
-        auto post_part = [&](auto cur_, auto prev_, int j) {
-            constexpr int CUR = decltype(cur_)::value, PREV = decltype(prev_)::value;
-            const unsigned char *w = lane_lds + (j & 3) * PART, *wn = lane_lds + ((j + 1) & 3) * PART;
-            const int last = p.post_parts - 1;
-            const int src2 = post_base + min(j + 2, last) * PART, dst2 = ((j + 2) & 3) * PART;
-#pragma unroll
-            for (int ks = 0; ks < 16; ++ks) {
-                const int sl = ks & 3, sn = (ks + 2) & 3;
-                if (ks == 14) {
-                    if (PREV) { if (S2D_FFN_POSTV) asm volatile("s_waitcnt vmcnt(20) lgkmcnt(0)" ::: "memory"); else asm volatile("s_waitcnt vmcnt(16) lgkmcnt(0)" ::: "memory"); }
-                    else asm volatile("s_waitcnt vmcnt(8) lgkmcnt(0)" ::: "memory");
-                    __builtin_amdgcn_s_barrier();
-                    __builtin_amdgcn_sched_barrier(0);
-                }
-                frag_read(sn, ks < 14 ? w + (2 * ks + 4) * FRAG : wn + (2 * (ks - 14)) * FRAG);
-                if (ks == 0) pm[CUR] = __builtin_amdgcn_mfma_f32_32x32x16_f16(fr[sl][0], xh[ks], zero16, 0, 0, 0); else mfma_a(pm[CUR], fr[sl][0], xh[ks]);
-                if (ks == 0 && PREV) add_load(j - 1, PREV == 1);
-                __builtin_amdgcn_sched_barrier(0);
-                if (ks == 0) px[CUR] = __builtin_amdgcn_mfma_f32_32x32x16_f16(fr[sl][0], xl[ks], zero16, 0, 0, 0); else mfma_a(px[CUR], fr[sl][0], xl[ks]);
-                auto piece = [&](int k) {
-                    const int s4 = src2 + (wave * 8 + (k & 4)) * FRAG, d4 = dst2 + (wave * 8 + (k & 4)) * FRAG;
-                    switch (k & 3) {
-                    case 0: dma_piece4(s4, d4, std::integral_constant<int, 0>{}); break;
-                    case 1: dma_piece4(s4, d4, std::integral_constant<int, 1>{}); break;
-                    case 2: dma_piece4(s4, d4, std::integral_constant<int, 2>{}); break;
-                    default: dma_piece4(s4, d4, std::integral_constant<int, 3>{}); break;
-                    }
-                };
-                if (S2D_FFN_POSTV) { if (ks < 4) piece(2 * ks); }
-                else if (ks < 8) piece(ks);
-                __builtin_amdgcn_sched_barrier(0);
-                mfma_a(px[CUR], fr[sl][1], xh[ks]);
-                if (S2D_FFN_POSTV && ks < 4) piece(2 * ks + 1);
-                if (PREV && ks >= 6 && ks < 14 && !(ks & 1)) tile_out(pm[CUR ^ 1], px[CUR ^ 1], j - 1, (ks - 6) >> 1);
-                __builtin_amdgcn_sched_barrier(0);
-            }
-        };
-        typedef std::integral_constant<int, 0> I0;
-        typedef std::integral_constant<int, 1> I1;
-        typedef std::integral_constant<int, 2> I2;
-        asm volatile("s_waitcnt vmcnt(0)" ::: "memory");
-        __syncthreads();
-        frag_read(0, lane_lds);
-        frag_read(1, lane_lds + 2 * FRAG);
+        const float *posr = p.post_pos + prow * p.post_ldpos + cb;
+        float *outr = p.post_out + rowc * p.post_ld + cb;
+        const float *pbr = p.post_bias + cb;
         const int npt = p.post_npos >> 5;
-        post_part(I0{}, I0{}, 0);
-        for (int j = 1; j < p.post_parts; ++j) {
+        for (int j = 0; j < p.post_parts; ++j) {
+#if S2D_FFN_DBG & 16
             if (j == 4) FFN_STAMP(13);
             if (j == 8) FFN_STAMP(14);
             if (j == 12) FFN_STAMP(15);
-            const bool hp = j - 1 < npt;
-            if (j & 1) { if (hp) post_part(I1{}, I1{}, j); else post_part(I1{}, I2{}, j); }
-            else { if (hp) post_part(I0{}, I1{}, j); else post_part(I0{}, I2{}, j); }
-        }
-        {
-            const int j = p.post_parts - 1;
-            add_load(j, j < npt);
-#pragma unroll
-            for (int q = 0; q < 4; ++q) { if (j & 1) tile_out(pm[1], px[1], j, q); else tile_out(pm[0], px[0], j, q); }
+#endif
+            const float *addr = (j < npt ? posr : pbr) + 32 * j;
+            const f32x4 a0 = *reinterpret_cast<const f32x4 *>(addr), a1 = *reinterpret_cast<const f32x4 *>(addr + 4);
+            const unsigned char *w = step_begin(n++);
+            f32x4 pm[2] = {zero4, zero4}, px[2] = {zero4, zero4};
+            xpart(w, pm, px);
+            f32x4 v0 = pm[0] + px[0] * (1.0f / 2048.0f), v1 = pm[1] + px[1] * (1.0f / 2048.0f);
+            v0 += a0; v1 += a1;
+            if (rowok) {
+                *reinterpret_cast<f32x4 *>(outr + 32 * j) = v0;
+                *reinterpret_cast<f32x4 *>(outr + 32 * j + 4) = v1;
+            }
         }
     }
 #if S2D_FFN_DBG & 16
@@ -725,8 +428,8 @@
     q.post_bias = post_bias; q.post_pos = post_npos > 0 ? post_pos : post_bias; q.post_out = post_out; q.post_parts = Npost / 32;
     q.pre_bias = pre_bias; q.pre_res = pre_res; q.site_pre = site_pre;
     q.post_S = post_npos > 0 ? post_S : 1; q.post_npos = post_npos; q.post_ld = (int)post_ld; q.post_ldpos = (int)post_ldpos;
-    const int smem = LDS_LN + 4 * FC * 4;
-    const dim3 grid(cdiv(M, 128)), block(256);
+    const int smem = LDS_ALL;
+    const dim3 grid(cdiv(M, ROWS_WG)), block(256);
     static S2dDevOnce attr[32];
     const bool drop = q.thresh != 0, ln1 = ln1_gamma != nullptr, ln2 = ln2_gamma != nullptr, post = Npost > 0, pre = pre_bias != nullptr;
     const void *fn = nullptr;
```

Result: slower. 173.8 clip-frames/s (-1.2%).
